# tsbertalan/openmg

Measured on AMD Instinct MI355X. Metric: V-cycles/sec, 3-D 7-point Poisson 256^3, higher is better.
Workload: dtype f64

## Files before the change

### include/openmg_hip.h

```cpp
#ifndef OPENMG_HIP_H
#define OPENMG_HIP_H

#include <stdint.h>

#ifdef __cplusplus
extern "C" {
#endif

#define OMG_OK                0
#define OMG_ERR_INVALID       1
#define OMG_ERR_NO_DEVICE     2
#define OMG_ERR_HIP           3
#define OMG_ERR_SINGULAR      4
#define OMG_ERR_NO_DIAGONAL   5
#define OMG_ERR_ALLOC         6
#define OMG_ERR_UNSUPPORTED   7

#define OMG_SMOOTH_GS_LEX     0
#define OMG_SMOOTH_GS_COLOUR  1
#define OMG_SMOOTH_JACOBI     2

typedef struct {
    int64_t n_rows, n_cols, nnz;
    const int32_t *indptr;
    const int32_t *indices;
    const double  *data;
} omg_csr;

typedef struct omg_hierarchy omg_hierarchy;
typedef struct omg_csr_result omg_csr_result;

const char *omg_last_error(void);
int omg_device_count(int *count);
int omg_set_device(int device);
int omg_device_mem_info(int64_t *free_bytes, int64_t *total_bytes);
int omg_device_synchronize(void);
const char *omg_version(void);

int omg_hierarchy_create(int n_levels, const omg_csr *A, const omg_csr *R,
                         int smoother, double omega, omg_hierarchy **out);
#define OMG_DTYPE_F64 0
#define OMG_DTYPE_F32 1
#define OMG_DTYPE_MIXED 2
int omg_hierarchy_create_ex(int n_levels, const omg_csr *A, const omg_csr *R, int smoother,
                            double omega, int dtype, omg_hierarchy **out);
int omg_hierarchy_create_from_fine(const omg_csr *A_in, int dim, const int64_t *shape, int n_restrictions, int smoother, double omega,
                                   int dtype, omg_hierarchy **out);

int omg_hierarchy_update_fine(omg_hierarchy *h, const double *data, int64_t nnz, int on_device);
int omg_hierarchy_dtype(const omg_hierarchy *h, int *dtype);
int omg_hierarchy_destroy(omg_hierarchy *h);
int omg_hierarchy_set_stream(omg_hierarchy *h, void *hip_stream);
int omg_hierarchy_sync(omg_hierarchy *h);
int omg_hierarchy_level_rows(const omg_hierarchy *h, int level, int64_t *n_rows);
int omg_hierarchy_level_sets(const omg_hierarchy *h, int level, int64_t *n_sets);
int omg_hierarchy_level_fused(const omg_hierarchy *h, int level, int *fused);
#define OMG_LEVEL_FUSED_LAST_SET   1
#define OMG_LEVEL_SCATTER_PROLONG  2
#define OMG_LEVEL_UNION_WALK       16
#define OMG_LEVEL_MARCH            32
#define OMG_LEVEL_MARCH_SCAN       512
#define OMG_LEVEL_PLANE            64
#define OMG_LEVEL_VAR7             256
#define OMG_LEVEL_STENCIL27        128
int omg_hierarchy_level_flags(const omg_hierarchy *h, int level, int *flags);
int omg_hierarchy_use_plane(omg_hierarchy *h, int enable);
#define OMG_CYCLE_V 0
#define OMG_CYCLE_F 1
#define OMG_CYCLE_W 2
int omg_hierarchy_set_cycle(omg_hierarchy *h, int shape, double over_correction);
int omg_hierarchy_get_cycle(const omg_hierarchy *h, int *shape, double *over_correction);
int omg_hierarchy_plane_info(const omg_hierarchy *h, int level, int64_t *out8);
int omg_hierarchy_set_info(const omg_hierarchy *h, int level, int set, int64_t *rows, int64_t *nnz);
#define OMG_FORMAT_FIELDS 12
int omg_hierarchy_format_info(const omg_hierarchy *h, int level, int op, int set, int64_t *out);
int omg_format_selftest(const omg_csr *A, int dtype, int64_t *out);

int omg_vcycle(omg_hierarchy *h, int level, const double *b, double *x,
               int pre, int post, double *norm);
int omg_vcycle_ex(omg_hierarchy *h, int level, const double *b, const double *x_in, double *x_out, double *x_pre,
                  int pre, int post, double *norm);

int omg_solve(omg_hierarchy *h, const double *b, double *x, int pre, int post,
              int max_cycles, double threshold, int *cycles_done, double *norm);

int omg_vcycle_dev(omg_hierarchy *h, int level, const double *b_dev, const double *x_in_dev, double *x_out_dev,
                   double *x_pre_dev, int pre, int post, double *norm);
int omg_resident_load_dev(omg_hierarchy *h, const double *b_dev, const double *x0_dev );
int omg_resident_fetch_dev(omg_hierarchy *h, double *x_dev);

int omg_hierarchy_cycle_dev(omg_hierarchy *h, const double *b_dev, double *x_dev, int pre, int post,
                            void *hip_stream);

int omg_resident_load(omg_hierarchy *h, const double *b, const double *x0 );
int omg_resident_cycle(omg_hierarchy *h, int pre, int post, double *norm );
int omg_resident_cycles(omg_hierarchy *h, int pre, int post, int n_cycles, double *norms );
int omg_resident_fetch(omg_hierarchy *h, double *x);
int omg_resident_spmv_time(omg_hierarchy *h, int reps, double *avg_ms);
int omg_resident_pcg(omg_hierarchy *h, int pre, int post, int max_iter, double threshold, int *iterations,
                     double *norms , double *true_norm, int *breakdown);
int omg_resident_use_graph(omg_hierarchy *h, int enable);

#define OMG_PROFILE_CLASSES 7
int omg_profile_enable(omg_hierarchy *h, int mask);
int omg_profile_read(omg_hierarchy *h, int64_t *launches, double *total_ms);

int omg_level_smooth(omg_hierarchy *h, int level, const double *b, double *x, int iterations);
int omg_level_residual(omg_hierarchy *h, int level, const double *b, const double *x,
                       double *r, double *norm );
int omg_level_spmv(omg_hierarchy *h, int level, const double *x, double *y);

int omg_level_restrict(omg_hierarchy *h, int level, const double *fine, double *coarse);
int omg_level_prolong_add(omg_hierarchy *h, int level, const double *coarse, double *fine_inout);
int omg_coarse_solve(omg_hierarchy *h, const double *b, double *x);
int omg_hierarchy_coarse_info(const omg_hierarchy *h, int64_t *out4);

int omg_spmv(const omg_csr *A, const double *x, double *y);
int omg_residual(const omg_csr *A, const double *b, const double *x, double *r, double *norm);
int omg_gauss_seidel(const omg_csr *A, const double *b, double *x, int smoother, double omega,
                     int iterations, double threshold, int *sweeps_done);
int omg_direct_solve(const omg_csr *A, const double *b, double *x);

int omg_rap(const omg_csr *R, const omg_csr *A, omg_csr_result **out,
            int64_t *n_rows, int64_t *n_cols, int64_t *nnz);
int omg_spgemm(const omg_csr *X, const omg_csr *Y, omg_csr_result **out,
               int64_t *n_rows, int64_t *n_cols, int64_t *nnz);
int omg_csr_result_fetch(omg_csr_result *res, int32_t *indptr, int32_t *indices, double *data);
int omg_csr_result_free(omg_csr_result *res);

int omg_restriction(int dim, const int64_t *shape, int32_t *indptr, int32_t *indices,
                    double *data, int64_t *n_rows, int64_t *nnz);

int omg_host_checksum(const void *buf, int64_t bytes, uint64_t *out);

typedef struct {
    omg_csr A;
    omg_csr R;
    int64_t n_halo;
    const int32_t *keys;
    int32_t n_sets;
    int32_t n_peers;
    const int32_t *peers;
    const int64_t *send_off;
    const int32_t *send_idx;
    const int64_t *recv_off;
    int32_t set_group;
    const int32_t *entry_group;
} omg_dist_level;
// ... 93 lines not shown
```

### openmg_amd/_hip.py

```python
import ctypes
import os

import numpy as np
import scipy.sparse as sp

_HERE = os.path.dirname(os.path.abspath(__file__))
LIB_PATH = os.environ.get("OMG_LIB_PATH") or os.path.join(_HERE, "lib", "libopenmg_hip.so")

OMG_OK = 0
ERR_INVALID, ERR_NO_DEVICE, ERR_HIP, ERR_SINGULAR, ERR_NO_DIAGONAL, ERR_ALLOC, ERR_UNSUPPORTED = range(1, 8)
SMOOTH_GS_LEX, SMOOTH_GS_COLOUR, SMOOTH_JACOBI = 0, 1, 2
PROFILE_CLASSES = 7
PROFILE_NAMES = ("smoother_set_sweep", "residual", "restrict", "prolong_add", "residual_norm", "plane_down", "plane_up")

SMOOTHERS = {
    "gs": SMOOTH_GS_LEX, "lex": SMOOTH_GS_LEX, "gauss-seidel": SMOOTH_GS_LEX, "gaussSeidel": SMOOTH_GS_LEX,
    "colour": SMOOTH_GS_COLOUR, "color": SMOOTH_GS_COLOUR, "rbgs": SMOOTH_GS_COLOUR,
    "red-black": SMOOTH_GS_COLOUR, "multicolour": SMOOTH_GS_COLOUR,
    "jacobi": SMOOTH_JACOBI, "weighted-jacobi": SMOOTH_JACOBI,
}


class HipError(RuntimeError):

    def __init__(self, code, message):
        super().__init__("libopenmg_hip: %s (code %d)" % (message, code))
        self.code = code


class CsrView(ctypes.Structure):
    _fields_ = [("n_rows", ctypes.c_int64), ("n_cols", ctypes.c_int64), ("nnz", ctypes.c_int64),
                ("indptr", ctypes.c_void_p), ("indices", ctypes.c_void_p), ("data", ctypes.c_void_p)]


_P = ctypes.c_void_p
_I = ctypes.c_int
_D = ctypes.c_double
_PP = ctypes.POINTER(ctypes.c_void_p)
_CSR = ctypes.POINTER(CsrView)
_I64P = ctypes.POINTER(ctypes.c_int64)
_IP = ctypes.POINTER(ctypes.c_int)
_DP = ctypes.POINTER(ctypes.c_double)

SIGNATURES = {
    "omg_last_error": (ctypes.c_char_p, []),
    "omg_version": (ctypes.c_char_p, []),
    "omg_device_count": (_I, [_IP]),
    "omg_set_device": (_I, [_I]),
    "omg_hierarchy_create": (_I, [_I, _CSR, _CSR, _I, _D, _PP]),
    "omg_hierarchy_create_ex": (_I, [_I, _CSR, _CSR, _I, _D, _I, _PP]),
    "omg_hierarchy_create_from_fine": (_I, [_CSR, _I, _I64P, _I, _I, _D, _I, _PP]),
    "omg_hierarchy_dtype": (_I, [_P, _IP]),
    "omg_hierarchy_update_fine": (_I, [_P, _P, ctypes.c_int64, _I]),
    "omg_hierarchy_destroy": (_I, [_P]),
    "omg_hierarchy_set_stream": (_I, [_P, _P]),
    "omg_hierarchy_sync": (_I, [_P]),
    "omg_hierarchy_level_rows": (_I, [_P, _I, _I64P]),
    "omg_hierarchy_level_sets": (_I, [_P, _I, _I64P]),
    "omg_hierarchy_set_info": (_I, [_P, _I, _I, _I64P, _I64P]),
    "omg_hierarchy_level_fused": (_I, [_P, _I, _IP]),
    "omg_hierarchy_level_flags": (_I, [_P, _I, _IP]),
    "omg_hierarchy_use_plane": (_I, [_P, _I]),
    "omg_hierarchy_set_cycle": (_I, [_P, _I, _D]),
    "omg_hierarchy_get_cycle": (_I, [_P, _IP, _DP]),
    "omg_hierarchy_plane_info": (_I, [_P, _I, _I64P]),
    "omg_hierarchy_format_info": (_I, [_P, _I, _I, _I, _I64P]),
    "omg_format_selftest": (_I, [_CSR, _I, _I64P]),
    "omg_vcycle": (_I, [_P, _I, _P, _P, _I, _I, _DP]),
    "omg_vcycle_ex": (_I, [_P, _I, _P, _P, _P, _P, _I, _I, _DP]),
    "omg_vcycle_dev": (_I, [_P, _I, _P, _P, _P, _P, _I, _I, _DP]),
    "omg_resident_load_dev": (_I, [_P, _P, _P]),
    "omg_resident_fetch_dev": (_I, [_P, _P]),
    "omg_device_synchronize": (_I, []),
    "omg_device_mem_info": (_I, [_I64P, _I64P]),
    "omg_solve": (_I, [_P, _P, _P, _I, _I, _I, _D, _IP, _DP]),
    "omg_resident_load": (_I, [_P, _P, _P]),
    "omg_resident_cycle": (_I, [_P, _I, _I, _DP]),
    "omg_resident_cycles": (_I, [_P, _I, _I, _I, _DP]),
    "omg_resident_fetch": (_I, [_P, _P]),
    "omg_resident_spmv_time": (_I, [_P, _I, _DP]),
    "omg_resident_use_graph": (_I, [_P, _I]),
    "omg_resident_pcg": (_I, [_P, _I, _I, _I, _D, _IP, _DP, _DP, _IP]),
    "omg_profile_enable": (_I, [_P, _I]),
    "omg_profile_read": (_I, [_P, _I64P, _DP]),
    "omg_level_smooth": (_I, [_P, _I, _P, _P, _I]),
    "omg_level_residual": (_I, [_P, _I, _P, _P, _P, _DP]),
    "omg_level_spmv": (_I, [_P, _I, _P, _P]),
    "omg_level_restrict": (_I, [_P, _I, _P, _P]),
    "omg_level_prolong_add": (_I, [_P, _I, _P, _P]),
    "omg_coarse_solve": (_I, [_P, _P, _P]),
    "omg_hierarchy_coarse_info": (_I, [_P, _I64P]),
    "omg_spmv": (_I, [_CSR, _P, _P]),
    "omg_residual": (_I, [_CSR, _P, _P, _P, _DP]),
    "omg_gauss_seidel": (_I, [_CSR, _P, _P, _I, _D, _I, _D, _IP]),
    "omg_direct_solve": (_I, [_CSR, _P, _P]),
    "omg_rap": (_I, [_CSR, _CSR, _PP, _I64P, _I64P, _I64P]),
    "omg_spgemm": (_I, [_CSR, _CSR, _PP, _I64P, _I64P, _I64P]),
    "omg_csr_result_fetch": (_I, [_P, _P, _P, _P]),
    "omg_csr_result_free": (_I, [_P]),
    "omg_restriction": (_I, [_I, _I64P, _P, _P, _P, _I64P, _I64P]),
    "omg_host_checksum": (_I, [_P, ctypes.c_int64, ctypes.POINTER(ctypes.c_uint64)]),
    "omg_dist_create": (_I, [_I, _I, _I, _P, _CSR, _I64P, _I, _D, _PP]),
    "omg_dist_create_ex": (_I, [_I, _I, _I, _P, _CSR, _I64P, _I, _D, _I, _PP]),
    "omg_dist_destroy": (_I, [_P]),
    "omg_dist_set_tail": (_I, [_P, _P]),
    "omg_hierarchy_cycle_dev": (_I, [_P, _P, _P, _I, _I, _P]),
    "omg_dist_set_stream": (_I, [_P, _P]),
    "omg_dist_sync": (_I, [_P]),
    "omg_rccl_unique_id": (_I, [_P]),
    "omg_rccl_self_exchange_time": (_I, [ctypes.c_int64, _I, _DP]),
    "omg_pdist_create": (_I, [_I, _I, _I, _I, _I, _I, _P, _D, _PP]),
    "omg_pdist_destroy": (_I, [_P]),
    "omg_pdist_set_tail": (_I, [_P, _P]),
    "omg_pdist_connect": (_I, [_P, _P, _P]),
    "omg_peer_access": (_I, [_I, _I, _P]),
    "omg_pdist_p2p_handle_count": (_I, [_P, _P]),
    "omg_pdist_p2p_handles": (_I, [_P, _P, _I]),
    "omg_pdist_p2p_open": (_I, [_P, _I, _P, _I]),
    "omg_pdist_p2p_local": (_I, [_P, _P]),
    "omg_pdist_p2p_enable": (_I, [_P, _I]),
    "omg_pdist_p2p_status": (_I, [_P, _P]),
    "omg_pdist_p2p_layout": (_I, [_P, _I64P, _I, _IP, _I]),
    "omg_pdist_cycles_squares": (_I, [_P, _I, _P]),
    "omg_pdist_rccl_ranks": (_I, [_P, _IP]),
    "omg_pdist_load": (_I, [_P, _P, _P]),
    "omg_pdist_fetch": (_I, [_P, _P]),
    "omg_pdist_sync": (_I, [_P]),
    "omg_pdist_info": (_I, [_P, _I64P]),
    "omg_pdist_set_gate": (_I, [_P, _I]),
    "omg_pdist_trace": (_I, [_P, _I]),
    "omg_pdist_progress": (_I, [_P, ctypes.POINTER(ctypes.c_uint)]),
    "omg_pdist_cycles": (_I, [_P, _I, _P]),
    "omg_pdist_cycles_ex": (_I, [_P, _I, _I, _I, _P]),
    "omg_pdist_group_cycles_ex": (_I, [_P, _I, _I, _I, _P]),
    "omg_sdist_p2p_handle_count": (_I, [_P, _P]),
    "omg_sdist_p2p_handles": (_I, [_P, _P, _I]),
    "omg_sdist_p2p_open": (_I, [_P, _I, _P, _I]),
    "omg_sdist_p2p_local": (_I, [_P, _P]),
    "omg_sdist_p2p_enable": (_I, [_P, _I]),
    "omg_sdist_p2p_status": (_I, [_P, _P]),
    "omg_sdist_p2p_layout": (_I, [_P, _I64P, _I, _IP]),
    "omg_pdist_group_create": (_I, [_I, _P, _PP]),
    "omg_pdist_group_destroy": (_I, [_P]),
    "omg_pdist_group_cycles": (_I, [_P, _I, _P]),
# ... 255 lines not shown
        check(lib().omg_resident_fetch_dev(self._h, ctypes.c_void_p(int(x_ptr))))

    def solve(self, b, x, pre, post, max_cycles, threshold):
        n = self.sizes[0]
        b = vec(b, n)
        assert x.dtype == np.float64 and x.flags.c_contiguous and x.size == n
        cycles = ctypes.c_int(0)
        norm = ctypes.c_double(0.0)
        check(lib().omg_solve(self._h, b.ctypes.data, x.ctypes.data, int(pre), int(post), int(max_cycles),
                              float(threshold), ctypes.byref(cycles), ctypes.byref(norm)))
        return cycles.value, norm.value

    def cycle_dev(self, b_dev, x_dev, pre, post, hip_stream=None):
        check(lib().omg_hierarchy_cycle_dev(self._h, ctypes.c_void_p(int(b_dev)), ctypes.c_void_p(int(x_dev)), int(pre), int(post),
                                            ctypes.c_void_p(hip_stream or 0)))

    def resident_load(self, b, x0=None):
        b = vec(b, self.sizes[0])
        x0 = None if x0 is None else vec(x0, self.sizes[0])
        check(lib().omg_resident_load(self._h, b.ctypes.data, None if x0 is None else x0.ctypes.data))

    def resident_cycle(self, pre, post, want_norm=True):
        if want_norm:
            norm = ctypes.c_double(0.0)
            check(lib().omg_resident_cycle(self._h, int(pre), int(post), ctypes.byref(norm)))
            return norm.value
        check(lib().omg_resident_cycle(self._h, int(pre), int(post), None))
        return None

    def resident_cycles(self, pre, post, n_cycles):
        norms = (ctypes.c_double * max(int(n_cycles), 1))()
        check(lib().omg_resident_cycles(self._h, int(pre), int(post), int(n_cycles), norms))
        return [float(norms[k]) for k in range(int(n_cycles))]

    def resident_fetch(self):
        x = np.empty(self.sizes[0], dtype=np.float64)
        check(lib().omg_resident_fetch(self._h, x.ctypes.data))
        return x

    def resident_pcg(self, pre, post, max_iter, threshold=0.0):
        max_iter = int(max_iter)
        if max_iter < 1:
            raise ValueError("max_iter must be >= 1")
        norms = np.zeros(max_iter, dtype=np.float64)
        it, tn, bd = ctypes.c_int(0), ctypes.c_double(0.0), ctypes.c_int(0)
        check(lib().omg_resident_pcg(self._h, int(pre), int(post), max_iter, float(threshold), ctypes.byref(it),
                                     norms.ctypes.data_as(_DP), ctypes.byref(tn), ctypes.byref(bd)))
        return int(it.value), norms[:it.value].copy(), float(tn.value), bool(bd.value)

    def spmv_time(self, reps=20):
        ms = ctypes.c_double(0.0)
        check(lib().omg_resident_spmv_time(self._h, int(reps), ctypes.byref(ms)))
        return ms.value

    def use_graph(self, enable=True):
        check(lib().omg_resident_use_graph(self._h, 1 if enable else 0))

    def set_stream(self, hip_stream):
        check(lib().omg_hierarchy_set_stream(self._h, ctypes.c_void_p(hip_stream or 0)))

    def sync(self):
        check(lib().omg_hierarchy_sync(self._h))

    def device_dtype(self):
        code = ctypes.c_int(-1)
        check(lib().omg_hierarchy_dtype(self._h, ctypes.byref(code)))
        return np.dtype(np.float32 if code.value in (DTYPE_F32, DTYPE_MIXED) else np.float64)

    def level_sets(self, level):
        v = ctypes.c_int64(0)
        check(lib().omg_hierarchy_level_sets(self._h, level, ctypes.byref(v)))
        return v.value

    def level_fused(self, level):
        v = ctypes.c_int(0)
        check(lib().omg_hierarchy_level_fused(self._h, level, ctypes.byref(v)))
        return bool(v.value)

    def level_flags(self, level):
        f = ctypes.c_int(0)
        check(lib().omg_hierarchy_level_flags(self._h, int(level), ctypes.byref(f)))
        return {"fused_last_set": bool(f.value & 1), "scatter_prolong": bool(f.value & 2), "union_walk": bool(f.value & 16),
                "march": bool(f.value & 32), "plane": bool(f.value & 64), "stencil27": bool(f.value & 128), "var7": bool(f.value & 256),
                "march_scan": bool(f.value & 512)}

    def use_plane(self, enable=True):
        check(lib().omg_hierarchy_use_plane(self._h, 1 if enable else 0))

    def set_cycle(self, shape="V", over_correction=1.0):
        check(lib().omg_hierarchy_set_cycle(self._h, cycle_code(shape), over_correction_of(over_correction)))

    def get_cycle(self):
        code, alpha = ctypes.c_int(-1), ctypes.c_double(0.0)
        check(lib().omg_hierarchy_get_cycle(self._h, ctypes.byref(code), ctypes.byref(alpha)))
        return {v: k for k, v in CYCLES.items()}[code.value], alpha.value

    PLANE_FIELDS = ("nx", "ny", "nz", "tile_x", "tile_y", "tile_z", "workgroups", "threads")

    def plane_info(self, level):
        out = (ctypes.c_int64 * len(self.PLANE_FIELDS))()
        check(lib().omg_hierarchy_plane_info(self._h, int(level), out))
        return dict(zip(self.PLANE_FIELDS, [int(v) for v in out]))

    def set_info(self, level, s):
        rows, nnz = ctypes.c_int64(0), ctypes.c_int64(0)
        check(lib().omg_hierarchy_set_info(self._h, level, s, ctypes.byref(rows), ctypes.byref(nnz)))
        return rows.value, nnz.value

    FORMAT_FIELDS = ("rows", "nnz", "blocks", "pattern_blocks", "pattern_rows", "pattern_nnz",
                     "coldict_nnz", "valdict_nnz", "format_bytes", "csr_bytes", "ell_blocks", "ell_nnz")

    def format_info(self, level, op="A", set=-1):
        out = (ctypes.c_int64 * len(self.FORMAT_FIELDS))()
        check(lib().omg_hierarchy_format_info(self._h, int(level), {"A": 0, "R": 1, "P": 2}[op], int(set), out))
        return dict(zip(self.FORMAT_FIELDS, [int(v) for v in out]))

    def profile_enable(self, classes=True):
        if classes is True:
            mask = -1
        elif not classes:
            mask = 0
        else:
            mask = 0
            for name in classes:
                mask |= 1 << PROFILE_NAMES.index(name)
        check(lib().omg_profile_enable(self._h, mask))

    def profile_read(self):
        n = (ctypes.c_int64 * PROFILE_CLASSES)()
        ms = (ctypes.c_double * PROFILE_CLASSES)()
        check(lib().omg_profile_read(self._h, n, ms))
        return {PROFILE_NAMES[i]: (int(n[i]), float(ms[i])) for i in range(PROFILE_CLASSES)}

    def smooth(self, level, b, x, iterations):
        n = self.sizes[level]
        b = vec(b, n)
        assert x.dtype == np.float64 and x.flags.c_contiguous and x.size == n
        check(lib().omg_level_smooth(self._h, level, b.ctypes.data, x.ctypes.data, int(iterations)))
        return x

    def residual(self, level, b, x, want_norm=False):
        n = self.sizes[level]
        b, x = vec(b, n), vec(x, n)
        r = np.empty(n)
        if want_norm:
            norm = ctypes.c_double(0.0)
            check(lib().omg_level_residual(self._h, level, b.ctypes.data, x.ctypes.data, r.ctypes.data, ctypes.byref(norm)))
            return r, norm.value
        check(lib().omg_level_residual(self._h, level, b.ctypes.data, x.ctypes.data, r.ctypes.data, None))
        return r

    def spmv(self, level, x):
        n = self.sizes[level]
        x = vec(x, n)
        y = np.empty(n)
        check(lib().omg_level_spmv(self._h, level, x.ctypes.data, y.ctypes.data))
        return y

    def restrict(self, level, fine):
        fine = vec(fine, self.sizes[level])
        out = np.empty(self.sizes[level + 1])
        check(lib().omg_level_restrict(self._h, level, fine.ctypes.data, out.ctypes.data))
        return out

    def prolong_add(self, level, coarse, fine):
        coarse = vec(coarse, self.sizes[level + 1])
        out = vec(fine, self.sizes[level], copy=True)
# ... 105 lines not shown
```

### openmg_amd/csrc/coarse.hip

```cpp
#include <algorithm>
#include <cmath>
#include <cstdlib>
#include <type_traits>

#include "common.h"

namespace omg {
namespace {

constexpr int64_t LDS_DOUBLES = 6144;

int grid1d(int64_t n, int cap = 65536) {
    int64_t g = (n + 255) / 256;
    if (g > cap) g = cap;
    if (g < 1) g = 1;
    return (int)g;
}

__device__ __forceinline__ double wsum(double v) {
#pragma unroll
    for (int off = 32; off > 0; off >>= 1) v += __shfl_down(v, off, 64);
    return v;
}
__device__ __forceinline__ float wsum(float v) {
#pragma unroll
    for (int off = 32; off > 0; off >>= 1) v += __shfl_down(v, off, 64);
    return v;
}

__global__ void couple_kernel(const double *B, int64_t m, const int32_t *cptr, const int32_t *cidx,
                              const double *cval, int64_t g, double *T) {
    const int64_t tot = m * g;
    for (int64_t t = blockIdx.x * (int64_t)blockDim.x + threadIdx.x; t < tot; t += (int64_t)gridDim.x * blockDim.x) {
        const int64_t i = t / g, c = t % g;
        double acc = 0.0;
        for (int32_t p = cptr[c]; p < cptr[c + 1]; ++p) acc += B[i * m + cidx[p]] * cval[p];
        T[t] = acc;
    }
}

__global__ void schur_kernel(const int32_t *rptr, const int32_t *ridx, const double *rval, int64_t g,
                             const double *T, double *S, int64_t ld) {
    const int64_t tot = g * g;
    for (int64_t t = blockIdx.x * (int64_t)blockDim.x + threadIdx.x; t < tot; t += (int64_t)gridDim.x * blockDim.x) {
        const int64_t q = t / g, c = t % g;
        double acc = 0.0;
        for (int32_t p = rptr[q]; p < rptr[q + 1]; ++p) acc += rval[p] * T[int64_t(ridx[p]) * g + c];
        if (acc != 0.0) S[q * ld + c] -= acc;
    }
}

template <typename V>
__global__ void narrow_kernel(const double *src, V *dst, int64_t n) {
    for (int64_t i = blockIdx.x * (int64_t)blockDim.x + threadIdx.x; i < n; i += (int64_t)gridDim.x * blockDim.x)
        dst[i] = V(src[i]);
}

template <typename V>
__global__ __launch_bounds__(256) void interior_solve_kernel(const V *__restrict__ binv, const int64_t *__restrict__ binv_off,
                                                             const int64_t *__restrict__ blk_off,
                                                             const int32_t *__restrict__ wg_blk, const int32_t *__restrict__ wg_row,
                                                             const int32_t *__restrict__ perm, const V *__restrict__ b,
                                                             V *__restrict__ y) {
    const int k = wg_blk[blockIdx.x];
    const int64_t o = blk_off[k], m = blk_off[k + 1] - o;
    const int64_t i = wg_row[blockIdx.x] + (threadIdx.x >> 6);
    if (i >= m) return;
    const int lane = threadIdx.x & 63;
    const V *row = binv + binv_off[k] + i * m;
    V acc = V(0);
    for (int64_t j = lane; j < m; j += 64) acc += row[j] * b[perm[o + j]];
    acc = wsum(acc);
    if (lane == 0) y[o + i] = acc;
}

template <typename V>
__global__ __launch_bounds__(256) void separator_solve_kernel(const V *__restrict__ sinv, int64_t g, int64_t n_int,
                                                              const int32_t *__restrict__ gptr, const int32_t *__restrict__ gidx,
                                                              const V *__restrict__ gval, const int32_t *__restrict__ perm,
                                                              const V *__restrict__ b, const V *__restrict__ y,
                                                              V *__restrict__ xg, V *__restrict__ x) {
    extern __shared__ unsigned char s_raw[];
    V *s_rhs = reinterpret_cast<V *>(s_raw);
    for (int64_t q = threadIdx.x; q < g; q += 256) {
        V acc = V(0);
        for (int32_t p = gptr[q]; p < gptr[q + 1]; ++p) acc += gval[p] * y[gidx[p]];
        s_rhs[q] = b[perm[n_int + q]] - acc;
    }
// ... 15 lines not shown
                                                               const int32_t *__restrict__ iptr, const int32_t *__restrict__ iidx,
                                                               const V *__restrict__ ival, const V *__restrict__ xg,
                                                               const int32_t *__restrict__ perm, const V *__restrict__ y,
                                                               int64_t w, V *__restrict__ x) {
    extern __shared__ unsigned char s_raw[];
    V *s_t = reinterpret_cast<V *>(s_raw);
    const int k = wg_blk[blockIdx.x];
    const int64_t o = blk_off[k], m = blk_off[k + 1] - o;
    const int64_t head = min(w, m), tail0 = max(head, m - w);
    const int64_t nt = head + (m - tail0);
    for (int64_t c = threadIdx.x; c < nt; c += 256) {
        const int64_t j = c < head ? c : tail0 + (c - head);
        V acc = V(0);
        for (int32_t p = iptr[o + j]; p < iptr[o + j + 1]; ++p) acc += ival[p] * xg[iidx[p]];
        s_t[c] = acc;
    }
    __syncthreads();
    const int64_t i = wg_row[blockIdx.x] + (threadIdx.x >> 6);
    if (i >= m) return;
    const int lane = threadIdx.x & 63;
    const V *row = binv + binv_off[k] + i * m;
    V acc = V(0);
    for (int64_t c = lane; c < nt; c += 64) {
        const int64_t j = c < head ? c : tail0 + (c - head);
        acc += row[j] * s_t[c];
    }
    acc = wsum(acc);
    if (lane == 0) x[perm[o + i]] = y[o + i] - acc;
}

constexpr int CHAIN_ROWS = 16;
template <typename V, bool BACK>
__global__ __launch_bounds__(256) void chain_step_kernel(const V *__restrict__ dinv, int64_t m, int64_t r0, const int32_t *__restrict__ ptr,
                                                         const int32_t *__restrict__ idx, const V *__restrict__ val,
                                                         const V *__restrict__ b, const V *src, V *z, V *x, int last) {
    extern __shared__ unsigned char s_raw[];
    V *s_t = reinterpret_cast<V *>(s_raw);
    for (int64_t q = threadIdx.x; q < m; q += 256) {
        V acc = V(0);
        for (int32_t p = ptr[r0 + q]; p < ptr[r0 + q + 1]; ++p) acc += val[p] * src[idx[p]];
        s_t[q] = BACK ? acc : b[r0 + q] - acc;
    }
    __syncthreads();
    const int lane = threadIdx.x & 63;
    const int64_t q0 = int64_t(blockIdx.x) * CHAIN_ROWS + (threadIdx.x >> 6) * 4;
    V acc[4] = {V(0), V(0), V(0), V(0)};
    const V *row[4];
#pragma unroll
    for (int r = 0; r < 4; ++r) row[r] = dinv + min(q0 + r, m - 1) * m;
    for (int64_t j = lane; j < m; j += 64) {
        const V t = s_t[j];
#pragma unroll
        for (int r = 0; r < 4; ++r) acc[r] += row[r][j] * t;
    }
#pragma unroll
    for (int r = 0; r < 4; ++r) {
        const V v = wsum(acc[r]);
        if (lane == 0 && q0 + r < m) {
            if (BACK) x[r0 + q0 + r] = z[r0 + q0 + r] - v;
            else { z[r0 + q0 + r] = v; if (last) x[r0 + q0 + r] = v; }
        }
    }
}

struct HostSub {
    std::vector<int32_t> ptr, idx;
    std::vector<double> val;
};

template <typename T, typename Al>
void put(DevBuf<T> &d, const std::vector<T, Al> &h, hipStream_t s) {
    d.alloc(std::max<size_t>(h.size(), 1));
    d.upload(h.data(), h.size(), s);
}

template <typename V>
void put_values(DevBuf<V> &d, const std::vector<double> &h, hipStream_t s, std::vector<V> &keep) {
    keep.assign(h.begin(), h.end());
    d.alloc(std::max<size_t>(keep.size(), 1));
    d.upload(keep.data(), keep.size(), s);
}

constexpr int SINE_THREADS = 1024;
typedef double v4d __attribute__((ext_vector_type(4)));
template <typename V, int E>
__global__ __launch_bounds__(SINE_THREADS) void sine_solve_kernel(const V *__restrict__ b, V *__restrict__ x, int nx, int ny, int nz,
                                                                 const double *__restrict__ tables, const double *__restrict__ lambda) {
    extern __shared__ double sine_buf[];
    const int px = nx + 1, n = nx * ny * nz;
    double *const lt = sine_buf + ((px * ny * nz + 1) & ~1);
    const int nt = (nx + ny + nz) * E;
    for (int r = int(threadIdx.x); r < nt; r += SINE_THREADS) lt[r] = tables[r];
    constexpr int PER = 8192 / SINE_THREADS;
    int place[PER];
    double lam[PER];
#pragma unroll
    for (int q = 0; q < PER; ++q) {
        const int r = int(threadIdx.x) + q * SINE_THREADS;
        place[q] = r < n ? (r / nx) * px + r % nx : -1;
        lam[q] = r < n ? lambda[r] : 1.0;
        if (r < n) sine_buf[place[q]] = double(b[r]);
    }
    __syncthreads();
    const int lane = int(threadIdx.x) & 63, wave = int(threadIdx.x) >> 6;
    const int c16 = lane & 15, k4 = lane >> 4;
#pragma unroll 1
    for (int pass = 0; pass < 6; ++pass) {
        const int axis = pass % 3;
        const int ne = axis == 0 ? nx : axis == 1 ? ny : nz;
        const int n_lines = n / ne;
        const int da = axis == 0 ? 1 : nx, sb = axis == 0 ? 0 : 1;
        const int sa = axis == 0 ? px : axis == 1 ? ny * px : px;
        const int stride = axis == 0 ? 1 : axis == 1 ? px : ny * px;
        const double *S = lt + (axis == 0 ? 0 : axis == 1 ? nx : nx + ny) * E;
        if (pass == 3) {
#pragma unroll
            for (int q = 0; q < PER; ++q)
                if (place[q] >= 0) sine_buf[place[q]] = sine_buf[place[q]] / lam[q];
            __syncthreads();
        }
        if (ne <= 1) continue;
        const int n_blocks = (n_lines + 15) >> 4, k_steps = (ne + 3) >> 2;
#pragma unroll 1
        for (int bl = wave; bl < n_blocks; bl += SINE_THREADS / 64) {
            const int line = 16 * bl + c16;
            const bool live = line < n_lines;
            const int bs = live ? (line / da) * sa + (line % da) * sb : 0;
            v4d acc[E / 16];
#pragma unroll
            for (int ib = 0; ib < E / 16; ++ib) acc[ib] = v4d{0.0, 0.0, 0.0, 0.0};
            double bvs[E / 4], avs[E / 16][E / 4];
#pragma unroll
            for (int ks = 0; ks < E / 4; ++ks) {
                const int k = 4 * ks + k4;
                bvs[ks] = (live && k < ne) ? sine_buf[bs + k * stride] : 0.0;
#pragma unroll
                for (int ib = 0; ib < E / 16; ++ib) avs[ib][ks] = S[(16 * ib + c16) * E + k];
            }
#pragma unroll
            for (int ks = 0; ks < E / 4; ++ks)
#pragma unroll
                for (int ib = 0; ib < E / 16; ++ib)
                    if (ks < k_steps) acc[ib] = __builtin_amdgcn_mfma_f64_16x16x4f64(avs[ib][ks], bvs[ks], acc[ib], 0, 0, 0);
            if (live) {
#pragma unroll
                for (int ib = 0; ib < E / 16; ++ib)
#pragma unroll
                    for (int r = 0; r < 4; ++r) {
                        const int i = 16 * ib + 4 * r + k4;
                        if (i < ne) sine_buf[bs + i * stride] = acc[ib][r];
                    }
            }
        }
        __syncthreads();
    }
#pragma unroll
    for (int q = 0; q < PER; ++q)
        if (place[q] >= 0) x[int(threadIdx.x) + q * SINE_THREADS] = V(sine_buf[place[q]]);
}

__device__ __forceinline__ void wave_lds_exchange() {
    __builtin_amdgcn_fence(__ATOMIC_RELEASE, "wavefront");
    __builtin_amdgcn_wave_barrier();
    __builtin_amdgcn_fence(__ATOMIC_ACQUIRE, "wavefront");
}

template <typename V>
__global__ __launch_bounds__(SINE_THREADS) void sine_cube16_kernel(const V *__restrict__ b, V *__restrict__ x, const double *__restrict__ tables,
                                                                   const double *__restrict__ lambda) {
    constexpr int N = 16, PX = N + 1;
    __shared__ double buf[N * N * PX];
    const int lane = int(threadIdx.x) & 63, w = int(threadIdx.x) >> 6;
    const int c = lane & 15, k4 = lane >> 4;
    double sx[4], sy[4], sz[4], lam[4], rhs[4];
#pragma unroll
    for (int ks = 0; ks < 4; ++ks) {
        sx[ks] = tables[(0 * N + c) * N + 4 * ks + k4];
        sy[ks] = tables[(1 * N + c) * N + 4 * ks + k4];
        sz[ks] = tables[(2 * N + c) * N + 4 * ks + k4];
        rhs[ks] = double(b[(w * N + c) * N + 4 * ks + k4]);
        lam[ks] = lambda[((4 * ks + k4) * N + w) * N + c];
    }
    auto transform = [&](const double (&S)[4], const double (&in)[4]) -> v4d {
        v4d acc = {0.0, 0.0, 0.0, 0.0};
#pragma unroll
        for (int ks = 0; ks < 4; ++ks) acc = __builtin_amdgcn_mfma_f64_16x16x4f64(S[ks], in[ks], acc, 0, 0, 0);
        return acc;
    };
    double in[4];
    v4d acc = transform(sx, rhs);
#pragma unroll
    for (int r = 0; r < 4; ++r) buf[(w * N + c) * PX + 4 * r + k4] = acc[r];
    wave_lds_exchange();
#pragma unroll
    for (int ks = 0; ks < 4; ++ks) in[ks] = buf[(w * N + 4 * ks + k4) * PX + c];
    acc = transform(sy, in);
#pragma unroll
    for (int r = 0; r < 4; ++r) buf[(w * N + 4 * r + k4) * PX + c] = acc[r];
    __syncthreads();
#pragma unroll
    for (int ks = 0; ks < 4; ++ks) in[ks] = buf[((4 * ks + k4) * N + w) * PX + c];
    acc = transform(sz, in);
#pragma unroll
    for (int r = 0; r < 4; ++r) in[r] = acc[r] / lam[r];
    acc = transform(sz, in);
#pragma unroll
    for (int r = 0; r < 4; ++r) buf[((4 * r + k4) * N + w) * PX + c] = acc[r];
    __syncthreads();
#pragma unroll
    for (int ks = 0; ks < 4; ++ks) in[ks] = buf[(w * N + c) * PX + 4 * ks + k4];
    acc = transform(sx, in);
#pragma unroll
    for (int r = 0; r < 4; ++r) buf[(w * N + c) * PX + 4 * r + k4] = acc[r];
    wave_lds_exchange();
#pragma unroll
    for (int ks = 0; ks < 4; ++ks) in[ks] = buf[(w * N + 4 * ks + k4) * PX + c];
    acc = transform(sy, in);
#pragma unroll
    for (int r = 0; r < 4; ++r) x[(w * N + 4 * r + k4) * N + c] = V(acc[r]);
}

bool detect_symmetric_star(const HostCsr &A, int64_t &nx, int64_t &ny, int64_t &nz, double (&c)[4]) {
    const int64_t n = A.n_rows;
    if (n < 2) return false;
    auto has = [&](int64_t r, int64_t col) {
        for (int32_t p = A.indptr[r]; p < A.indptr[r + 1]; ++p)
            if (A.indices[p] == col) return true;
        return false;
    };
    nx = n;
    for (int64_t r = 1; r < n; ++r)
        if (!has(r, r - 1)) { nx = r; break; }
    if (nx < 2 || n % nx) return false;
    const int64_t lines = n / nx;
    ny = lines;
    for (int64_t q = 1; q < lines; ++q)
        if (!has(q * nx, (q - 1) * nx)) { ny = q; break; }
    if (lines % ny) return false;
    nz = lines / ny;
    const int64_t sj = nx, sk = nx * ny;
    bool have[4] = {false, false, false, false};
    c[0] = c[1] = c[2] = c[3] = 0.0;
    for (int64_t r = 0; r < n; ++r) {
        const int64_t i = r % nx, jl = (r / nx) % ny, kl = r / sk;
        const int want = 1 + (i > 0) + (i + 1 < nx) + (jl > 0) + (jl + 1 < ny) + (kl > 0) + (kl + 1 < nz);
        if (A.indptr[r + 1] - A.indptr[r] != want) return false;
        int seen = 0;
        for (int32_t p = A.indptr[r]; p < A.indptr[r + 1]; ++p) {
            const int64_t off = int64_t(A.indices[p]) - r;
            int slot, bit;
            if (off == 0) { slot = 0; bit = 1; }
            else if (off == -1 && i > 0) { slot = 1; bit = 2; }
            else if (off == 1 && i + 1 < nx) { slot = 1; bit = 4; }
            else if (off == -sj && jl > 0 && ny > 1) { slot = 2; bit = 8; }
            else if (off == sj && jl + 1 < ny) { slot = 2; bit = 16; }
            else if (off == -sk && kl > 0 && nz > 1) { slot = 3; bit = 32; }
            else if (off == sk && kl + 1 < nz) { slot = 3; bit = 64; }
            else return false;
            if (seen & bit) return false;
            seen |= bit;
            if (!have[slot]) { have[slot] = true; c[slot] = A.data[p]; }
            else if (A.data[p] != c[slot]) return false;
        }
    }
    return have[0];
}

}

template <typename V>
void CoarseSolver<V>::build(const HostCsr &A, hipStream_t s) {
    OMG_REQUIRE(A.n_rows == A.n_cols, "coarse operator must be square");
    n = A.n_rows;
    if (n == 0) return;
    {
        const char *e = getenv("OMG_COARSE_BLOCKS"), *q = getenv("OMG_COARSE_SINE");
        if (!(e && atoi(e) > 0) && !(q && q[0] == '0') && build_sine(A, s)) return;
    }
    int64_t band = 0;
    for (int64_t i = 0; i < n; ++i)
        for (int32_t p = A.indptr[i]; p < A.indptr[i + 1]; ++p) band = std::max<int64_t>(band, std::llabs(int64_t(A.indices[p]) - i));
    w = std::max<int64_t>(band, 1);
    const int64_t lds_cap = LDS_DOUBLES * int64_t(sizeof(double) / sizeof(V));
    P = 1;
    {
        const char *e = getenv("OMG_COARSE_BLOCKS");
        const int forced = e ? atoi(e) : 0;
        const bool big = double(n) * double(n) * sizeof(V) > double(size_t(256) << 20);
        double best = double(n) * double(n);
        if (forced > 1 || (forced == 0 && big))
            for (int q = 2; q <= 64; ++q) {
                const int64_t gq = int64_t(q - 1) * w;
                if (gq >= n || gq > lds_cap || 2 * w > lds_cap) break;
                const int64_t mq = (n - gq + q - 1) / q;
                if (mq < 2 * w) break;
                const double cost = double(q) * double(mq) * double(mq) + double(gq) * double(gq);
                if ((forced == q) || (forced == 0 && cost < best)) { best = cost; P = q; }
                if (forced == q) break;
            }
    }
    std::vector<int32_t> plain_ptr(A.indptr.begin(), A.indptr.end());
    DevBuf<int32_t> d_ptr, d_idx;
// ... 196 lines not shown
    DevBuf<double> c_val, r_val;
    for (int k = 0; k < K; ++k) {
        const int64_t r0 = int64_t(k) * bs, m = std::min(n, r0 + bs) - r0;
        if (k > 0) for (int64_t i = r0 - bs; i < r0; ++i) rmap[size_t(i)] = -1;
        for (int64_t i = 0; i < m; ++i) rmap[size_t(r0 + i)] = int32_t(i);
        d_rmap.upload(rmap.data(), size_t(n), s);
        OMG_HIP(hipStreamSynchronize(s));
        fill_augmented_from_csr(d_ptr, d_idx, d_val, n, d_rmap.p, d_rmap.p, m, W.p, s);
        if (k > 0) {
            const int64_t p0 = r0 - bs, mp = bs;
            HostSub col, row;
            std::vector<std::vector<std::pair<int32_t, double>>> cols{size_t(m)};
            for (int64_t r = p0; r < r0; ++r)
                for (int32_t p = up.ptr[size_t(r)]; p < up.ptr[size_t(r) + 1]; ++p) cols[size_t(up.idx[size_t(p)] - r0)].emplace_back(int32_t(r - p0), up.val[size_t(p)]);
            col.ptr.assign(size_t(m) + 1, 0);
            for (int64_t c = 0; c < m; ++c) {
                for (auto &e : cols[size_t(c)]) { col.idx.push_back(e.first); col.val.push_back(e.second); }
                col.ptr[size_t(c) + 1] = int32_t(col.idx.size());
            }
            row.ptr.assign(size_t(m) + 1, 0);
            for (int64_t q = 0; q < m; ++q) {
                for (int32_t p = lo.ptr[size_t(r0 + q)]; p < lo.ptr[size_t(r0 + q) + 1]; ++p) { row.idx.push_back(int32_t(lo.idx[size_t(p)] - p0)); row.val.push_back(lo.val[size_t(p)]); }
                row.ptr[size_t(q) + 1] = int32_t(row.idx.size());
            }
            put(c_ptr, col.ptr, s); put(c_idx, col.idx, s); put(c_val, col.val, s);
            put(r_ptr, row.ptr, s); put(r_idx, row.idx, s); put(r_val, row.val, s);
            hipLaunchKernelGGL(couple_kernel, dim3(grid1d(mp * m)), dim3(256), 0, s, inv64.p, mp, c_ptr.p, c_idx.p, c_val.p, m, T.p);
            hipLaunchKernelGGL(schur_kernel, dim3(grid1d(m * m)), dim3(256), 0, s, r_ptr.p, r_idx.p, r_val.p, m, T.p, W.p, 2 * m);
            OMG_HIP(hipGetLastError());
        }
        gauss_jordan_inverse(W.p, m, inv64.p, s, keep.p);
        hipLaunchKernelGGL((narrow_kernel<V>), dim3(grid1d(m * m)), dim3(256), 0, s, inv64.p, dinv.p + size_t(k) * size_t(bs) * size_t(bs), m * m);
        OMG_HIP(hipGetLastError());
        OMG_HIP(hipStreamSynchronize(s));
    }
    if (lds_need > size_t(48) << 10) {
        OMG_HIP(hipFuncSetAttribute(reinterpret_cast<const void *>(chain_step_kernel<V, false>), hipFuncAttributeMaxDynamicSharedMemorySize, int(lds_need)));
        OMG_HIP(hipFuncSetAttribute(reinterpret_cast<const void *>(chain_step_kernel<V, true>), hipFuncAttributeMaxDynamicSharedMemorySize, int(lds_need)));
    }
    bytes = (size_t(2 * K - 1) * size_t(bs) * size_t(bs)) * sizeof(V);
}

template <typename V>
bool CoarseSolver<V>::build_sine(const HostCsr &A, hipStream_t s) {
    int64_t gx = 0, gy = 0, gz = 0;
    double c[4];
    if (A.n_rows > 8192 || !detect_symmetric_star(A, gx, gy, gz, c) || gx > 32 || gy > 32 || gz > 32) return false;
    const double pi = 3.14159265358979323846264338327950288;
    const int64_t E = std::max(gx, std::max(gy, gz)) <= 16 ? 16 : 32;
    std::vector<double> tab(size_t((gx + gy + gz) * E), 0.0), lam(size_t(A.n_rows));
    auto table = [&](double *t, int64_t m) {
        const long double f = std::sqrt(2.0L / (long double)(m + 1));
        for (int64_t i = 0; i < m; ++i)
            for (int64_t p = 0; p < m; ++p)
                t[i * E + p] = m == 1 ? 1.0 : double(f * sinl((long double)pi * (long double)((i + 1) * (p + 1)) / (long double)(m + 1)));
    };
    table(tab.data(), gx);
    table(tab.data() + gx * E, gy);
    table(tab.data() + (gx + gy) * E, gz);
    double smallest = 1e300, largest = 0.0;
    for (int64_t r = 0; r < A.n_rows; ++r) {
        const int64_t p = r % gx, q = (r / gx) % gy, t = r / (gx * gy);
        double l = c[0] + 2.0 * c[1] * std::cos(pi * double(p + 1) / double(gx + 1));
        if (gy > 1) l += 2.0 * c[2] * std::cos(pi * double(q + 1) / double(gy + 1));
        if (gz > 1) l += 2.0 * c[3] * std::cos(pi * double(t + 1) / double(gz + 1));
        lam[size_t(r)] = l;
        smallest = std::min(smallest, std::fabs(l));
        largest = std::max(largest, std::fabs(l));
    }
    if (!(smallest > 1e-13 * largest)) return false;
    P = 0;
    sx = int(gx); sy = int(gy); sz = int(gz);
    sine.alloc(tab.size());
    lambda.alloc(lam.size());
    sine.upload(tab.data(), tab.size(), s);
    lambda.upload(lam.data(), lam.size(), s);
    OMG_HIP(hipStreamSynchronize(s));
    w = gx * gy;
    bytes = (tab.size() + lam.size()) * sizeof(double);
    return true;
}

template <typename V>
void CoarseSolver<V>::solve(const V *b, V *x, hipStream_t s) const {
    if (n == 0) return;
    if (P == 0) {
        const int E = std::max(sx, std::max(sy, sz)) <= 16 ? 16 : 32;
        const size_t lds = (size_t(sx + 1) * size_t(sy) * size_t(sz) + 2 + size_t(sx + sy + sz) * size_t(E)) * sizeof(double);
        static const bool cube16 = [] { const char *e = experiment_env("OMG_SINE_CUBE16"); return !(e && e[0] == '0'); }();
        if (E == 16 && sx == 16 && sy == 16 && sz == 16 && cube16) {
            hipLaunchKernelGGL((sine_cube16_kernel<V>), dim3(1), dim3(SINE_THREADS), 0, s, b, x, sine.p, lambda.p);
        } else if (E == 16) {
            hipLaunchKernelGGL((sine_solve_kernel<V, 16>), dim3(1), dim3(SINE_THREADS), lds, s, b, x, sx, sy, sz, sine.p, lambda.p);
        } else {
            if (lds > size_t(64) * 1024)
                OMG_HIP(hipFuncSetAttribute(reinterpret_cast<const void *>(sine_solve_kernel<V, 32>), hipFuncAttributeMaxDynamicSharedMemorySize, int(lds)));
            hipLaunchKernelGGL((sine_solve_kernel<V, 32>), dim3(1), dim3(SINE_THREADS), lds, s, b, x, sx, sy, sz, sine.p, lambda.p);
        }
        OMG_HIP(hipGetLastError());
        return;
    }
    if (P == 1) {
        launch_dense_gemv<V>(inv.p, b, x, n, s);
        return;
    }
    if (P == -1) {
        for (int k = 0; k < K; ++k) {
            const int64_t r0 = int64_t(k) * bs, m = std::min(n, r0 + bs) - r0;
            hipLaunchKernelGGL((chain_step_kernel<V, false>), dim3(unsigned((m + CHAIN_ROWS - 1) / CHAIN_ROWS)), dim3(256), size_t(m) * sizeof(V), s,
                               dinv.p + size_t(k) * size_t(bs) * size_t(bs), m, r0, lo_ptr.p, lo_idx.p, lo_val.p, b, z.p, z.p, x, k == K - 1 ? 1 : 0);
        }
        for (int k = K - 2; k >= 0; --k) {
            const int64_t r0 = int64_t(k) * bs;
            hipLaunchKernelGGL((chain_step_kernel<V, true>), dim3(unsigned((bs + CHAIN_ROWS - 1) / CHAIN_ROWS)), dim3(256), size_t(bs) * sizeof(V), s,
                               dinv.p + size_t(k) * size_t(bs) * size_t(bs), bs, r0, up_ptr.p, up_idx.p, up_val.p, b, x, z.p, x, 0);
        }
        OMG_HIP(hipGetLastError());
        return;
    }
    hipLaunchKernelGGL((interior_solve_kernel<V>), dim3((unsigned)n_wg), dim3(256), 0, s, binv.p, binv_off.p, blk_off.p,
                       wg_blk.p, wg_row.p, perm.p, b, y.p);
    hipLaunchKernelGGL((separator_solve_kernel<V>), dim3((unsigned)((g + 3) / 4)), dim3(256), (size_t)(g) * sizeof(V), s,
                       sinv.p, g, n_int, gi_ptr.p, gi_idx.p, gi_val.p, perm.p, b, y.p, xg.p, x);
    hipLaunchKernelGGL((interior_correct_kernel<V>), dim3((unsigned)n_wg), dim3(256), (size_t)(2 * w) * sizeof(V), s, binv.p,
                       binv_off.p, blk_off.p, wg_blk.p, wg_row.p, ig_ptr.p, ig_idx.p, ig_val.p, xg.p, perm.p, y.p, w, x);
    OMG_HIP(hipGetLastError());
}

template struct CoarseSolver<double>;
template struct CoarseSolver<float>;

}
```

### openmg_amd/csrc/common.h

```cpp
#pragma once
#include <hip/hip_runtime.h>

#include <algorithm>
#include <array>
#include <cstdint>
#include <cstdio>
#include <cstdlib>
#include <cstring>
#include <new>
#include <stdexcept>
#include <memory>
#include <string>
#include <type_traits>
#include <utility>
#include <vector>

#include "../../include/openmg_hip.h"

#if !defined(OMG_EXPERIMENTS) && (defined(PLANE_STORE_AUX) || defined(PLANE_LA_BIG) || defined(PLANE_LA) || defined(PLANE_WAVE_SYNC) || \
                                  defined(PLANE_WSYNC_F32) || defined(S27_COEF_AUX) || defined(S27_SG) || defined(S27_WAVES) ||        \
                                  defined(MARCH_NAP_MAX) || defined(OMG_ROWBLK_NNZ) || defined(PLANE_SETPRIO))
#error "tuning switches are experiments: add -DOMG_EXPERIMENTS"
#endif

// ... 395 lines not shown
};

template <typename V>
struct RowArgsT {
    const V *x = nullptr;
    const V *b = nullptr;
    V *y = nullptr;
    double omega = 1.0;
    double *partials = nullptr;
    V *zero = nullptr;
    const int32_t *ymap = nullptr;
    const V *first_diag = nullptr;
    int first_end = 0;
    bool first_jacobi = false;
    const RowValues<V> *values = nullptr;
};
using RowArgs = RowArgsT<double>;

template <typename V>
void launch_rows(const DevCsrT<V> &A, int mode, int set, const RowArgsT<V> &args, hipStream_t s);
template <typename V>
void launch_rows_range(const DevCsrT<V> &A, int mode, int set_begin, int set_end, const RowArgsT<V> &args,
                       hipStream_t s);
template <typename V>
void launch_gs_serial(const DevCsrT<V> &A, int set_begin, int set_end, const RowArgsT<V> &args,
                      hipStream_t s);
constexpr int SUM_FOLD = 64;
void launch_sum(double *partials, int64_t n, double *out, hipStream_t s);
void launch_sum_sqrt(double *partials, int64_t n, double *out, hipStream_t s);
void launch_sum_batch(const double *partials, int64_t stride, int64_t n, int count, double *out, bool take_sqrt,
                      hipStream_t s);
template <typename S, typename D>
void launch_gather(const S *src, const int32_t *idx, D *dst, int64_t n, hipStream_t s);
template <typename S, typename D>
void launch_scatter(const S *src, const int32_t *idx, D *dst, int64_t n, hipStream_t s);
template <typename V>
void launch_diagonal(const DevCsrT<V> &A, V *diag, hipStream_t s);
template <typename V>
void launch_scale_values(const V *in, V *out, int64_t n, double factor, hipStream_t s);
template <typename V>
void launch_first_relaxation(const V *b, const V *diag, V *x, int64_t n, int64_t first_end, bool jacobi, double omega,
                             hipStream_t s);
template <typename V>
void launch_dense_gemv(const V *M, const V *v, V *out, int64_t n, hipStream_t s);
template <typename V>
void launch_dense_gemv_rows(const V *M, const V *v, V *out, int64_t rows, int64_t n,
                            hipStream_t s);
void dense_inverse_from_csr(const DevCsr &A, double *Minv, hipStream_t s);
void gauss_jordan_inverse(double *W, int64_t n, double *Minv, hipStream_t s, double *keep_ws = nullptr);
void fill_augmented_from_csr(const int32_t *indptr, const int32_t *indices, const double *data, int64_t n_rows,
                             const int32_t *rmap, const int32_t *cmap, int64_t m, double *W, hipStream_t s);

template <typename V>
struct CoarseSolver {
    int64_t n = 0;
    int P = 1;
    DevBuf<V> inv;
    int64_t n_int = 0, g = 0, w = 0;
    DevBuf<V> binv, sinv;
    DevBuf<int64_t> blk_off, binv_off;
    DevBuf<int32_t> perm;
    DevBuf<int32_t> wg_blk, wg_row;
    int64_t n_wg = 0;
    DevBuf<int32_t> gi_ptr, gi_idx;
    DevBuf<V> gi_val;
    DevBuf<int32_t> ig_ptr, ig_idx;
    DevBuf<V> ig_val;
    DevBuf<V> y, xg;
    int sx = 0, sy = 0, sz = 0;
    DevBuf<double> sine, lambda;
    size_t bytes = 0;
    bool retain_workspace = false;
    DevBuf<double> ws_aug, ws_inv64, ws_keep;
    int64_t bs = 0;
    int K = 0;
    DevBuf<V> dinv;
    DevBuf<int32_t> lo_ptr, lo_idx, up_ptr, up_idx;
    DevBuf<V> lo_val, up_val;
    DevBuf<V> z;
    void build_chain(const HostCsr &A, const int32_t *d_ptr, const int32_t *d_idx, const double *d_val, hipStream_t s);
    void build(const HostCsr &A, hipStream_t s);
    bool build_sine(const HostCsr &A, hipStream_t s);
    void solve(const V *b, V *x, hipStream_t s) const;
};

constexpr int MARCH_FACE_PAD = 72;
struct MarchGeom {
    int nx = 0, ny = 0, nz = 0;
    int TJ = 0, TK = 0;
    int ntj = 0, ntk = 0, n_tiles = 0;
    int T = 0, n_grp = 0;
    int n_pat = 0;
};
template <typename V>
struct MarchPlan {
    MarchGeom g;
    DevBuf<uint32_t> codes;
    DevBuf<V> coef;
    DevBuf<uint32_t> sync;
    DevBuf<int32_t> order;
    DevBuf<V> faceJ, faceK;
    bool line1 = false;
    DevBuf<V> tri;
    bool per_row = false;
    DevBuf<V> rowc;
    bool line_scan = false;
    int scan_c = 0, scan_g = 0;
    DevBuf<uint8_t> rowcode;
    DevBuf<V> face_scan;
    bool build(const omg_csr &A, hipStream_t s);
    void sweep(V *x, const V *b, hipStream_t s) const;
    bool timed_out(hipStream_t s) const;
};

struct DevCsrPlain {
    int64_t n_rows = 0, n_cols = 0, nnz = 0;
    DevBuf<int32_t> indptr, indices;
    DevBuf<double> data;
};
void galerkin_chain_device(const omg_csr &A0, int dim, const int64_t *shape, int n_restrictions, std::vector<DevCsrPlain> &A,
                           std::vector<DevCsrPlain> &R, hipStream_t s);
HostCsr download_csr(const DevCsrPlain &M, hipStream_t s);
bool rap_aggregation_device(const DevCsrPlain &R, const DevCsrPlain &A, DevCsrPlain &C, hipStream_t s);

bool is_plain_aggregation(const omg_csr &R, int64_t nx, int64_t ny, int64_t nz, double &w);

constexpr int PLANE_EDGE = 4;
struct PlaneGeom {
    int nx = 0, ny = 0, nz = 0;
    int hx = 0;
    int z_base = 0, z_end = 0, kv0 = 0, kv1 = 0, kc_off = 0, nzc = 0;
    int TX = 0, TY = 0, LZ = 0;
    int PX = 0, PY = 0;
    int ntx = 0, nty = 0, ntz = 0, n_wg = 0;
    int threads = 0;
    size_t lds_bytes = 0;
    double c[7] = {0, 0, 0, 0, 0, 0, 0};
    double w = 0.0;
    double over = 1.0;
    bool dim2 = false;
    bool jacobi = false;
    double omega = 1.0;
    bool block = false;
    bool la2 = true;
};
template <typename V>
struct PlanePlan {
    PlaneGeom g;
    DevBuf<double> partials;
    uint32_t *status = nullptr;
    bool build(const omg_csr &A, const omg_csr &R, Ordering &ord, bool jacobi = false, double omega = 1.0);
    bool build_device(const DevCsrPlain &A, int nx, int ny, int nz, double w, Ordering &ord, bool jacobi, double omega, hipStream_t s);
    bool finish_geometry(int64_t nx, int64_t ny, int64_t nz, const double (&c)[7], double w, bool jacobi, double omega);
    void spmv(const V *x, V *y, hipStream_t s) const;
    HostCsr operator_csr() const;
    HostCsr restriction_csr() const;
    void build_slab(int nx, int ny, int nz_own, int ghost, int ghost_c, bool first, bool last, const double (&c)[7], double w);
    struct Peer {
        V *x[2] = {nullptr, nullptr};
        V *bc[2] = {nullptr, nullptr};
        int64_t shift = 0, cshift = 0;
        int planes = 0, cplanes = 0;
        int zc_lo = 0, zc_hi = 0;
        const uint32_t *wait_flag[4] = {nullptr, nullptr, nullptr, nullptr};
        uint32_t wait_seq[4] = {0, 0, 0, 0};
        bool fused_wait = true;
        uint32_t *done = nullptr;
        uint32_t *flag[2] = {nullptr, nullptr};
        uint32_t seq = 0;
        uint32_t *status = nullptr;
        uint32_t spin = 1u << 21;
    };
    struct Coarse {
        const int32_t *map = nullptr;
        V *b = nullptr;
        V *x = nullptr;
        const V *diag = nullptr;
        int first_end = 0;
        const V *e = nullptr;
    };
    void tune(V *x, V *tmp, const V *b, const Coarse &c, hipStream_t s, bool finest = true);
    float time_pair(V *x, V *tmp, const V *b, const Coarse &c, hipStream_t s, bool finest, int pairs);
    enum { PART_ALL = 0, PART_EDGE = 1, PART_INNER = 2 };
    bool can_split() const {
        return !g.dim2 && !g.block && !(g.la2 && g.threads <= 128) && (g.z_end - g.z_base) >= 3 * PLANE_EDGE;
    }
    int split_partials() const {
        const int nzo = g.z_end - g.z_base;
        return nzo >= 3 * PLANE_EDGE ? g.ntx * g.nty * (2 + (nzo - 2 * PLANE_EDGE + g.LZ - 1) / g.LZ) : g.n_wg;
    }
    struct Gate {
        const uint32_t *flag[4] = {nullptr, nullptr, nullptr, nullptr};
        uint32_t seq[4] = {0, 0, 0, 0};
        uint32_t *status = nullptr;
        uint32_t spin = 1u << 21;
    };
    bool can_gate() const { return can_split() && 2 * g.ntx * g.nty <= 192 && (g.z_end - g.z_base) >= 96; }
    int gate_lz() const;
    int gate_partials() const;
    void down(const V *x_old, V *x_new, const V *b, bool x_zero, const Coarse &c, hipStream_t s, const Peer *peer = nullptr,
              bool sweep = true, int part = PART_ALL, const Gate *gate = nullptr) const;
    void up(const V *x_old, V *x_new, const V *b, const Coarse &c, double *out, hipStream_t s, const Peer *peer = nullptr,
            bool sweep = true, int part = PART_ALL, const Gate *gate = nullptr) const;
};

template <typename V>
struct Var7Plan {
    int nx = 0, ny = 0, nz = 0;
    double w = 0.0;
    double over = 1.0;
    bool sym = false;
    int tx = 0, ty = 0, lz = 0, ntx = 0, nty = 0, ntz = 0, threads = 0;
    int64_t n_wg = 0;
    DevBuf<V> cD, cM[3], cP[3];
    DevBuf<double> partials;
    bool build(const omg_csr &A, const omg_csr &R, Ordering &ord, hipStream_t s);
    bool build_device(const DevCsrPlain &A, int nx, int ny, int nz, double w, Ordering &ord, hipStream_t s);
    HostCsr operator_csr(hipStream_t s) const;
    HostCsr restriction_csr() const;
    struct Coarse {
        const int32_t *map = nullptr;
        V *b = nullptr;
        const V *e = nullptr;
    };
    void down(const V *x_old, V *x_new, const V *b, bool x_zero, const Coarse &c, hipStream_t s, bool sweep = true) const;
    void up(const V *x_old, V *x_new, const V *b, const Coarse &c, double *out, hipStream_t s, bool sweep = true) const;
    void rap_from(const int32_t *indptr, const double *vals, bool write_fine, double *coarse_dense, Var7Plan<V> *coarse,
                  unsigned long long *err, hipStream_t s);
};

template <typename V>
void var7_rap(const int32_t *indptr, const double *vals, int nx, int ny, int nz, double w, Var7Plan<V> *fine, Var7Plan<V> *coarse,
              double *coarse_dense, unsigned long long *err, hipStream_t s);

struct S27Geom {
    int nx = 0, ny = 0, nz = 0;
    int hx = 0, hy = 0, hz = 0;
    int64_t na = 0;
    int rg = 0;
    int L = 0, G = 0;
    int64_t nl = 0, ng = 0;
    int wpb = 4;
    int n_wg = 0;
    double w = 0.0;
    double over = 1.0;
};
template <typename V>
struct Stencil27Plan {
    S27Geom g;
    DevBuf<V> coef;
    DevBuf<V> res67;
    DevBuf<double> partials;
    bool have67 = false;
    int64_t live_lo = 0, live_hi = 0, live_lo01 = 0, live_hi01 = 0;
    bool build(const omg_csr &A, const omg_csr &R, Ordering &ord, hipStream_t s);
    bool build_device(const DevCsrPlain &A, int nx, int ny, int nz, double w, Ordering &ord, hipStream_t s);
    void build_slab(const DevCsrPlain &A, int nx, int ny, int nz_ext, bool first, bool last, double w, hipStream_t s);
    bool tile(const DevCsrPlain &A, const S27Geom &q, int kz_lo, int kz_hi, int kb_lo, int kb_hi, hipStream_t s);
    size_t plane_rows_count() const;
    void pack_plane_rows(int K, V *buf, hipStream_t s) const;
    void unpack_plane_rows(int K, const V *buf, hipStream_t s);
    void sweep(const V *x_old, V *x_new, const V *b, bool x_zero, double *norm_old, bool last, double *norm_new, hipStream_t s);
    void place_tiles(V *x, V *tmp, V *b, hipStream_t s);
    void residual_restrict(const V *x, const V *b, bool use67, const int32_t *cmap, V *bc, hipStream_t s);
    void norm(const V *x, const V *b, bool use67, double *out, hipStream_t s);
    void prolong(V *x, const V *e, const int32_t *cmap, hipStream_t s);
    HostCsr operator_csr(hipStream_t s) const;
    HostCsr restriction_csr() const;
    void rap_from(const int32_t *indptr, const double *vals, bool write_fine, double *coarse_dense, Stencil27Plan<V> *coarse, hipStream_t s);
};

enum { PCG_RHO = 0, PCG_ALPHA = 1, PCG_BETA = 2, PCG_DONE = 3, PCG_BREAK = 4, PCG_ITERS = 5, PCG_NSC = 8 };
constexpr int PCG_MAX_WG = 2048;
struct PcgPlane {
    int nx, ny, nz, hx;
    int64_t nr;
    double c[7];
};
template <typename V>
int pcg_wgs(int64_t n);
template <typename V, typename Z>
void pcg_dots(const V *r, const Z *z, const V *q, int64_t n, double *part, const double *sc, hipStream_t s);
template <typename V>
void pcg_dot(const V *a, const V *b, int64_t n, double *part, const double *sc, hipStream_t s);
template <typename V, typename Z>
void pcg_pupdate(const Z *z, const V *p, V *p2, int64_t n, const double *sc, hipStream_t s);
template <typename V, typename Z>
void pcg_update(V *x, const V *p, V *r, const V *q, Z *rlo, int64_t n, double *part, const double *sc, hipStream_t s);
template <typename V, typename Z>
// ... 14 lines not shown
```

### openmg_amd/csrc/hierarchy.hip

```cpp
#include <algorithm>
#include <chrono>
#include <cmath>
#include <cstring>
#include <memory>
#include <array>
#include <map>
#include <mutex>
#include <thread>
#include <type_traits>

#include "common.h"

namespace omg {

std::vector<ScatteredBlock> &scattered_registry() {
    static std::vector<ScatteredBlock> r;
    return r;
}
static std::mutex &scattered_mutex() {
    static std::mutex m;
    return m;
}
static void scattered_release(ScatteredBlock &blk, size_t mapped) {
    auto report = [](const char *what, hipError_t e) {
// ... 81 lines not shown
                    "no HIP device visible: libopenmg_hip.so has no CPU fallback "
                    "(hipGetDeviceCount: " + std::string(hipGetErrorString(e)) + ")");
}

namespace {

inline bool getenv_flag(const char *name) { const char *e = getenv(name); return e && e[0] == '1'; }
inline bool getenv_flag0(const char *name) { const char *e = getenv(name); return e && e[0] == '0'; }

struct SweepStep {
    int set_begin, set_end;
    bool serial;
};

template <typename V>
struct Level {
    int64_t n = 0;
    DevCsrT<V> A;
    DevCsrT<V> R;
    DevCsrT<V> P;
    Ordering ord;
    DevBuf<int32_t> perm;
    DevBuf<int32_t> r_out;
    DevBuf<V> x, b, r, tmp;
    DevBuf<V> diag;
    DevBuf<double> partials;
    DevBuf<double> nat;
    V *xp = nullptr, *tp = nullptr;
    std::vector<SweepStep> plan;
    bool scatter_prolong = false;
    DevBuf<V> pw_data, pw_vdict, pw_pval, pw_vell;
    RowValues<V> pw;
    double pw_factor = 0.0;
    std::unique_ptr<MarchPlan<V>> march;
    std::unique_ptr<PlanePlan<V>> plane;
    std::unique_ptr<Stencil27Plan<V>> s27;
    std::unique_ptr<Var7Plan<V>> var7;
    DevBuf<char> pool;
    size_t pool_span = 0, pool_off1 = 0, pool_off2 = 0;
    DevBuf<V> spmv_y;
    bool format_pending = false;
};

struct ProfEvent {
    int cls;
    hipEvent_t a, b;
};

template <typename V>
struct Hier {
    using value_type = V;
    std::vector<Level<V>> lv;
    CoarseSolver<V> coarse;
    DevBuf<double> norm_dev;
    DevBuf<uint32_t> plane_status;
    DevBuf<V> pre_buf;
    int pre_level = -1;
    DevBuf<double> norms_dev;
    DevBuf<double> batch_partials;
    DevBuf<V> pcg_b, pcg_x, pcg_p, pcg_p2, pcg_q;
    DevBuf<double> pcg_sc, pcg_part, pcg_norms;
    bool mixed = false;
    struct Mixed {
        bool plane = false;
        PcgPlane pg{};
        DevCsrT<double> A;
        DevBuf<int32_t> src;
        DevBuf<double> b, x, x2, r, p, p2, q;
    } mx;
    int smoother = OMG_SMOOTH_GS_LEX;
    double omega = 1.0;
    int cycle_shape = OMG_CYCLE_V;
    double over = 1.0;
    hipStream_t own = nullptr, stream = nullptr;
    DevBuf<int32_t> indptr0;
    int64_t nnz0 = 0;
    std::vector<DevBuf<double>> dense27;
    bool upd7 = false;
    int g7[3] = {0, 0, 0};
    std::vector<DevBuf<double>> dense7;
    bool resident = false;
    bool no_fuse = [] { const char *e = getenv("OMG_NO_FUSE"); return e && e[0] == '1'; }();
    bool no_plane = false;
    struct GraphSlot {
        hipGraphExec_t exec = nullptr;
        int pre = -1, post = -1;
        std::vector<V *> before, after;
    };
    bool want_graph = false;
    std::vector<GraphSlot> graphs;
    unsigned profiling = 0;
    std::vector<ProfEvent> events;
    int64_t prof_n[OMG_PROFILE_CLASSES] = {0};
    double prof_ms[OMG_PROFILE_CLASSES] = {0};
    std::vector<hipEvent_t> event_pool;

    Hier() = default;
    Hier(const Hier &) = delete;
    Hier &operator=(const Hier &) = delete;
    ~Hier() {
        for (auto &g : graphs) if (g.exec) (void)hipGraphExecDestroy(g.exec);
        for (auto &e : events) { (void)hipEventDestroy(e.a); (void)hipEventDestroy(e.b); }
        for (auto &e : event_pool) (void)hipEventDestroy(e);
        if (own) (void)hipStreamDestroy(own);
    }
};

}
}

struct omg_hierarchy {
    std::unique_ptr<omg::Hier<double>> d;
    std::unique_ptr<omg::Hier<float>> f;
};

namespace omg {
namespace {

void check_diagonal(const omg_csr &A, int level) {
    const int64_t bad = first_row_without_diagonal(A);
    if (bad >= 0)
        throw Error(OMG_ERR_NO_DIAGONAL, "level " + std::to_string(level) + ": row " +
                                             std::to_string(bad) + " has no nonzero diagonal entry");
}

omg_csr view(const HostCsr &A) {
    return omg_csr{A.n_rows, A.n_cols, A.nnz, A.indptr.data(), A.indices.data(), A.data.data()};
}

template <typename V>
void order_level(Level<V> &L, const omg_csr &A, int smoother, hipStream_t s) {
    L.march.reset();
    if (smoother == OMG_SMOOTH_GS_LEX && !getenv_flag0("OMG_MARCH")) {
        std::unique_ptr<MarchPlan<V>> plan(new MarchPlan<V>);
        if (plan->build(A, s)) {
            L.march = std::move(plan);
            L.ord = Ordering();
            L.ord.identity = true;
            L.ord.sets = {0, A.n_rows};
            return;
        }
    }
    L.ord = make_ordering(A, smoother);
}

template <typename V>
void build_plan(Level<V> &L) {
    L.plan.clear();
    const int ns = (int)L.A.n_sets();
    int s = 0;
    while (s < ns) {
        auto one_block = [&](int k) { return L.A.set_blk[k + 1] - L.A.set_blk[k] == 1; };
        if (one_block(s)) {
            int e = s + 1;
            while (e < ns && one_block(e)) ++e;
            L.plan.push_back({s, e, e - s >= 2});
            s = e;
        } else {
            L.plan.push_back({s, s + 1, false});
            ++s;
        }
    }
}

template <typename V>
struct Prof {
    Hier<V> *h;
    int idx = -1;
    Prof(Hier<V> *hh, int level, int cls) : h(hh) {
        if (level != 0 || !((h->profiling >> cls) & 1u)) return;
// ... 320 lines not shown
    }
    L.x.zero(h->stream); L.tmp.zero(h->stream); L.b.zero(h->stream); C.x.zero(h->stream);
    L.xp = L.x.p;
    L.tp = L.tmp.p;
    OMG_HIP(hipStreamSynchronize(h->stream));
}

template <typename V>
void place_s27_tiles(Hier<V> *h) {
    if (h->lv.size() < 2) return;
    Level<V> &L = h->lv[0];
    if (!L.s27 || !L.tmp.p || L.n < POOL_TRIAL_MIN) return;
    L.s27->place_tiles(L.x.p, L.tmp.p, L.b.p, h->stream);
    L.x.zero(h->stream); L.tmp.zero(h->stream); L.b.zero(h->stream);
    OMG_HIP(hipStreamSynchronize(h->stream));
}

template <typename V>
void ensure_spmv_y(Hier<V> *h, Level<V> &L) {
    if (L.spmv_y.p) return;
    L.spmv_y.alloc(size_t(L.n));
    static const int trials = [] { const char *e = getenv("OMG_SPMV_TRIALS"); return e && e[0] ? atoi(e) : 16; }();
    if (trials < 2 || !L.plane || L.n < POOL_TRIAL_MIN) return;
    hipEvent_t e0, e1;
    OMG_HIP(hipEventCreate(&e0));
    OMG_HIP(hipEventCreate(&e1));
    auto timed = [&]() -> float {
        L.plane->spmv(L.xp, L.spmv_y.p, h->stream);
        OMG_HIP(hipEventRecord(e0, h->stream));
        for (int r = 0; r < 8; ++r) L.plane->spmv(L.xp, L.spmv_y.p, h->stream);
        OMG_HIP(hipEventRecord(e1, h->stream));
        OMG_HIP(hipEventSynchronize(e1));
        float ms = 0.0f;
        OMG_HIP(hipEventElapsedTime(&ms, e0, e1));
        return 1e3f * ms / 8.0f;
    };
    float best = timed(), worst = best;
    const bool debug = SetupTimer::on();
    if (debug) fprintf(stderr, "[omg setup] SpMV destination, candidate 0: %.1f us per launch\n", best);
    std::vector<DevBuf<V>> held;
    for (int k = 1; k < trials; ++k) {
        if (2.0 * double(sizeof(V)) * double(L.n) / (double(best) * 1e-6) >= 5.15e12) break;
        DevBuf<V> alt;
        try { alt.alloc(size_t(L.n), 0, pool_placement(k)); } catch (const Error &) { (void)hipGetLastError(); break; }
        std::swap(L.spmv_y, alt);
        const float t = timed();
        if (debug) fprintf(stderr, "[omg setup] SpMV destination, candidate %d (placement %d): %.1f us per launch\n", k, pool_placement(k), t);
        worst = std::max(worst, t);
        if (t < best) best = t;
        else std::swap(L.spmv_y, alt);
        held.push_back(std::move(alt));
    }
    (void)hipEventDestroy(e0);
    (void)hipEventDestroy(e1);
}

template <typename V>
bool use_s27(const Hier<V> *h, const Level<V> &L) {
    return L.s27 && !h->no_plane;
}

template <typename V>
bool use_var7(const Hier<V> *h, const Level<V> &L) {
    return L.var7 && !h->no_plane;
}

template <typename V>
bool use_plane(const Hier<V> *h, const Level<V> &L, int pre, int post) {
    (void)pre; (void)post;
    return L.plane && !h->no_plane;
}

template <typename V>
int cycle_body(Hier<V> *h, int l, int pre, int post, bool want_norm = false, double *pre_slot = nullptr,
               bool first_done = false, double *post_slot = nullptr, bool x_zero = false, int shape = -1);

template <typename V>
void cycle_children(Hier<V> *h, int l, int pre, int post, int shape, bool first_done, bool x_zero) {
    cycle_body(h, l + 1, pre, post, false, nullptr, first_done, nullptr, x_zero, shape);
    if (shape != OMG_CYCLE_V && l + 1 < (int)h->lv.size() - 1)
        cycle_body(h, l + 1, pre, post, false, nullptr, false, nullptr, false, shape == OMG_CYCLE_F ? OMG_CYCLE_V : OMG_CYCLE_W);
}

template <typename V>
int cycle_body(Hier<V> *h, int l, int pre, int post, bool want_norm, double *pre_slot, bool first_done, double *post_slot, bool x_zero,
               int shape) {
    if (shape < 0) shape = h->cycle_shape;
    const int last = (int)h->lv.size() - 1;
    if (l >= last) {
        coarse_solve_level(h);
        return NORM_NONE;
    }
    Level<V> &L = h->lv[l];
    Level<V> &C = h->lv[l + 1];
    if (use_s27(h, L)) {
        Stencil27Plan<V> &P = *L.s27;
        const bool child_zero = l + 1 < last && ((use_s27(h, C) && pre >= 1) || (use_plane(h, C, pre, post) && pre == 1));
        bool zero_now = x_zero;
        if (x_zero && pre == 0) {
            OMG_HIP(hipMemsetAsync(L.xp, 0, size_t(L.n) * sizeof(V), h->stream));
            zero_now = false;
        }
        for (int it = 0; it < pre; ++it) {
            Prof<V> p(h, l, 0);
            P.sweep(L.xp, L.tp, L.b.p, zero_now, (it == 0 && !zero_now) ? pre_slot : nullptr, it + 1 == pre, nullptr, h->stream);
            std::swap(L.xp, L.tp);
            zero_now = false;
        }
        if (l == h->pre_level) OMG_HIP(hipMemcpyAsync(h->pre_buf.p, L.xp, size_t(L.n) * sizeof(V), hipMemcpyDeviceToDevice, h->stream));
        if (l + 1 < last && !child_zero) OMG_HIP(hipMemsetAsync(C.xp, 0, size_t(C.n) * sizeof(V), h->stream));
        {
            Prof<V> p(h, l, 1);
            P.residual_restrict(L.xp, L.b.p, pre >= 1, L.r_out.p, C.b.p, h->stream);
        }
        cycle_children(h, l, pre, post, shape, false, child_zero);
        {
            Prof<V> p(h, l, 3);
            P.prolong(L.xp, C.xp, L.r_out.p, h->stream);
        }
        double *nslot = want_norm ? (post_slot ? post_slot : P.partials.p) : nullptr;
        for (int it = 0; it < post; ++it) {
            Prof<V> p(h, l, 0);
            const bool fin = it + 1 == post && want_norm;
            P.sweep(L.xp, L.tp, L.b.p, false, nullptr, fin, fin ? nslot : nullptr, h->stream);
            std::swap(L.xp, L.tp);
        }
        return want_norm ? NORM_S27 : NORM_NONE;
    }
    static const int halves = [] { const char *e = experiment_env("OMG_PLANE_HALVES"); return (e && (e[0] == '1' || e[0] == '2')) ? e[0] - '0' : 3; }();
    if (use_plane(h, L, pre, post) && halves == 2 && !x_zero && pre >= 1 && post >= 1) {
        const bool res_done = smooth_level(h, l, pre, FUSE_RESIDUAL, nullptr, first_done);
        residual_level(h, l, L.r.p, res_done);
        if (l + 1 < last) ensure_format(h, l + 1);
        const bool child_first = l + 1 < last && first_sweep_in_restrict(h, C, pre);
        restrict_level<V>(h, l, L.r.p, C.b.p, l + 1 < last ? C.xp : nullptr, child_first);
        cycle_children(h, l, pre, post, shape, child_first, false);
        typename PlanePlan<V>::Coarse c;
        c.map = L.r_out.p;
        c.e = C.xp;
        double *out = (want_norm && post == 1) ? (post_slot ? post_slot : L.plane->partials.p) : nullptr;
        L.plane->up(L.xp, L.tp, L.b.p, c, out, h->stream);
        std::swap(L.xp, L.tp);
        if (post > 1)
            return smooth_level(h, l, post - 1, want_norm ? FUSE_NORM : FUSE_NONE, nullptr, false, post_slot) ? NORM_LAST_SET : NORM_NONE;
        return out ? NORM_PLANE : NORM_NONE;
    }
    if (use_plane(h, L, pre, post) && halves == 1 && pre >= 1 && post >= 1) {
        if (pre > 1) smooth_level(h, l, pre - 1, FUSE_NONE, nullptr, first_done);
        if (l + 1 < last) ensure_format(h, l + 1);
        const bool child_first = l + 1 < last && first_sweep_in_restrict(h, C, pre);
        typename PlanePlan<V>::Coarse c;
        c.map = L.r_out.p;
        c.b = C.b.p;
        c.x = l + 1 < last ? C.xp : nullptr;
        c.diag = child_first ? C.diag.p : nullptr;
        c.first_end = child_first ? int(C.A.sets[1]) : 0;
        L.plane->down(L.xp, L.tp, L.b.p, x_zero, c, h->stream);
        std::swap(L.xp, L.tp);
        cycle_children(h, l, pre, post, shape, child_first, false);
        prolong_add_level<V>(h, l, C.xp, L.xp, h->over);
        return smooth_level(h, l, post, want_norm ? FUSE_NORM : FUSE_NONE, nullptr, false, post_slot) ? NORM_LAST_SET : NORM_NONE;
    }
    if (use_plane(h, L, pre, post)) {
        if (pre > 1) smooth_level(h, l, pre - 1, FUSE_NONE, nullptr, first_done);
        const bool child_plane = l + 1 < last && use_plane(h, C, pre, post);
        const bool child_zero = child_plane && pre <= 1 && halves == 3;
        if (l + 1 < last && !child_zero) ensure_format(h, l + 1);
        const bool child_first = l + 1 < last && !child_zero && !use_s27(h, C) && !L.plane->g.dim2 && first_sweep_in_restrict(h, C, pre);
        typename PlanePlan<V>::Coarse c;
        c.map = L.r_out.p;
        c.b = C.b.p;
        c.x = (l + 1 < last && !child_zero) ? C.xp : nullptr;
        c.diag = child_first ? C.diag.p : nullptr;
        c.first_end = child_first ? int(C.A.sets[1]) : 0;
        if (child_zero && pre == 0) OMG_HIP(hipMemsetAsync(C.xp, 0, size_t(C.n) * sizeof(V), h->stream));
        {
            Prof<V> p(h, l, 5);
            L.plane->down(L.xp, L.tp, L.b.p, x_zero, c, h->stream, nullptr, pre >= 1);
        }
        if (pre >= 1) std::swap(L.xp, L.tp);
        if (l == h->pre_level) OMG_HIP(hipMemcpyAsync(h->pre_buf.p, L.xp, size_t(L.n) * sizeof(V), hipMemcpyDeviceToDevice, h->stream));
        cycle_children(h, l, pre, post, shape, child_first, child_zero);
        c.e = C.xp;
        double *out = (want_norm && post <= 1) ? (post_slot ? post_slot : L.plane->partials.p) : nullptr;
        {
            Prof<V> p(h, l, 6);
            L.plane->up(L.xp, L.tp, L.b.p, c, out, h->stream, nullptr, post >= 1);
        }
        std::swap(L.xp, L.tp);
        if (post > 1)
            return smooth_level(h, l, post - 1, want_norm ? FUSE_NORM : FUSE_NONE, nullptr, false, post_slot) ? NORM_LAST_SET : NORM_NONE;
        return out ? NORM_PLANE : NORM_NONE;
    }
    if (use_var7(h, L)) {
        Var7Plan<V> &P = *L.var7;
        if (pre > 1) smooth_level(h, l, pre - 1, FUSE_NONE, nullptr, first_done);
        const bool child_zero = l + 1 < last && ((use_var7(h, C) && pre == 1) || (use_plane(h, C, pre, post) && pre == 1) || (use_s27(h, C) && pre >= 1));
        if (l + 1 < last && !child_zero) {
            if (!use_s27(h, C)) ensure_format(h, l + 1);
            OMG_HIP(hipMemsetAsync(C.xp, 0, size_t(C.n) * sizeof(V), h->stream));
        }
        typename Var7Plan<V>::Coarse c;
        c.map = L.r_out.p;
        c.b = C.b.p;
        {
            Prof<V> p(h, l, 5);
            P.down(L.xp, L.tp, L.b.p, x_zero && pre == 1, c, h->stream, pre >= 1);
        }
        if (pre >= 1) std::swap(L.xp, L.tp);
        else if (x_zero) OMG_HIP(hipMemsetAsync(L.xp, 0, size_t(L.n) * sizeof(V), h->stream));
        if (l == h->pre_level) OMG_HIP(hipMemcpyAsync(h->pre_buf.p, L.xp, size_t(L.n) * sizeof(V), hipMemcpyDeviceToDevice, h->stream));
        cycle_children(h, l, pre, post, shape, false, child_zero);
        c.e = C.xp;
        double *out = (want_norm && post <= 1) ? (post_slot ? post_slot : P.partials.p) : nullptr;
        {
            Prof<V> p(h, l, 6);
            P.up(L.xp, L.tp, L.b.p, c, out, h->stream, post >= 1);
        }
        std::swap(L.xp, L.tp);
        if (post > 1)
            return smooth_level(h, l, post - 1, want_norm ? FUSE_NORM : FUSE_NONE, nullptr, false, post_slot) ? NORM_LAST_SET : NORM_NONE;
        return out ? NORM_VAR7 : NORM_NONE;
    }
    const bool res_done = smooth_level(h, l, pre, FUSE_RESIDUAL, pre_slot, first_done);
    if (l == h->pre_level) OMG_HIP(hipMemcpyAsync(h->pre_buf.p, L.xp, size_t(L.n) * sizeof(V), hipMemcpyDeviceToDevice, h->stream));
    residual_level(h, l, L.r.p, res_done);
    const bool child_zero = l + 1 < last && ((use_plane(h, C, pre, post) && pre == 1 && halves == 3) || (use_s27(h, C) && pre >= 1));
    if (l + 1 < last && !child_zero && !use_s27(h, C)) ensure_format(h, l + 1);
    const bool child_first = l + 1 < last && !child_zero && !use_s27(h, C) && !use_var7(h, C) && first_sweep_in_restrict(h, C, pre);
    restrict_level<V>(h, l, L.r.p, C.b.p, (l + 1 < last && !child_zero) ? C.xp : nullptr, child_first);
    cycle_children(h, l, pre, post, shape, child_first, child_zero);
    prolong_add_level<V>(h, l, C.xp, L.xp, h->over);
    if (post > 0)
        return smooth_level(h, l, post, want_norm ? FUSE_NORM : FUSE_NONE, nullptr, false, post_slot) ? NORM_LAST_SET : NORM_NONE;
    return NORM_NONE;
}

template <typename V>
void finish_norm(Hier<V> *h, int l, int state, double *out = nullptr) {
    if (state == NORM_PLANE) {
        Level<V> &L = h->lv[l];
        launch_sum_sqrt(L.plane->partials.p, L.plane->g.n_wg, out ? out : h->norm_dev.p, h->stream);
    } else if (state == NORM_VAR7) {
        Level<V> &L = h->lv[l];
        launch_sum_sqrt(L.var7->partials.p, L.var7->n_wg, out ? out : h->norm_dev.p, h->stream);
    } else if (state == NORM_S27) {
        Level<V> &L = h->lv[l];
        Stencil27Plan<V> &P = *L.s27;
        {
            Prof<V> p(h, l, 4);
            P.norm(L.xp, L.b.p, P.have67, P.partials.p, h->stream);
        }
        launch_sum_sqrt(P.partials.p, int64_t(4) * P.g.n_wg, out ? out : h->norm_dev.p, h->stream);
    } else {
        norm_level<V>(h, l, nullptr, state == NORM_LAST_SET, out);
    }
}

template <typename V>
constexpr bool direct_io(const Level<V> &L) { return std::is_same<V, double>::value && L.ord.identity; }

template <typename V>
void ensure_nat(Hier<V> *h, int l) {
    Level<V> &L = h->lv[l];
    if (!direct_io(L) && L.nat.n < size_t(std::max<int64_t>(L.n, 1))) L.nat.alloc(std::max<int64_t>(L.n, 1));
}

// ... 23 lines not shown
        if (L.march && L.march->timed_out(h->stream))
            throw Error(OMG_ERR_HIP, "lexicographic wavefront sweep timed out waiting for a neighbouring tile's face; the iterate and "
                                     "the hand-over slots of this hierarchy are no longer consistent: destroy it and build a new one");
    if (h->plane_status.p && !have_plane_status) {
        OMG_HIP(hipMemcpyAsync(&plane_st, h->plane_status.p, sizeof(plane_st), hipMemcpyDeviceToHost, h->stream));
        OMG_HIP(hipStreamSynchronize(h->stream));
    }
    check_plane_status(h, plane_st);
}

template <typename V>
void fetch_vec(Hier<V> *h, int l, const V *src, double *host) {
    Level<V> &L = h->lv[l];
    if (direct_io(L)) {
        download_staged(host, src, size_t(L.n) * sizeof(double), h->stream);
    } else {
        ensure_nat(h, l);
        launch_scatter<V, double>(src, L.ord.identity ? nullptr : L.perm.p, L.nat.p, L.n, h->stream);
        download_staged(host, L.nat.p, size_t(L.n) * sizeof(double), h->stream);
    }
    check_march(h);
}

template <typename V>
void load_vec_dev(Hier<V> *h, int l, const double *dev, V *dst) {
    Level<V> &L = h->lv[l];
    if (direct_io(L)) OMG_HIP(hipMemcpyAsync(dst, dev, L.n * sizeof(double), hipMemcpyDeviceToDevice, h->stream));
    else launch_gather<double, V>(dev, L.ord.identity ? nullptr : L.perm.p, dst, L.n, h->stream);
}
template <typename V>
void fetch_vec_dev(Hier<V> *h, int l, const V *src, double *dev) {
    Level<V> &L = h->lv[l];
    if (direct_io(L)) OMG_HIP(hipMemcpyAsync(dev, src, L.n * sizeof(double), hipMemcpyDeviceToDevice, h->stream));
    else launch_scatter<V, double>(src, L.ord.identity ? nullptr : L.perm.p, dev, L.n, h->stream);
}

template <typename V>
double read_norm(Hier<V> *h) {
    double v = 0.0;
    uint32_t st = 0;
    OMG_HIP(hipMemcpyAsync(&v, h->norm_dev.p, sizeof(double), hipMemcpyDeviceToHost, h->stream));
    if (h->plane_status.p) OMG_HIP(hipMemcpyAsync(&st, h->plane_status.p, sizeof(st), hipMemcpyDeviceToHost, h->stream));
    OMG_HIP(hipStreamSynchronize(h->stream));
    check_march(h, true, st);
    return v;
}

template <typename V>
void drop_graph(Hier<V> *h) {
    for (auto &g : h->graphs) if (g.exec) (void)hipGraphExecDestroy(g.exec);
    h->graphs.clear();
}

template <typename V>
std::vector<V *> pointer_state(const Hier<V> *h) {
    std::vector<V *> s;
    s.reserve(2 * h->lv.size());
    for (const Level<V> &L : h->lv) { s.push_back(L.xp); s.push_back(L.tp); }
    return s;
}

template <typename V>
void run_cycle0(Hier<V> *h, int pre, int post) {
    const bool single = h->lv.size() == 1;
    auto body = [&]() {
        const int part = cycle_body(h, 0, pre, post, !single);
        if (!single) finish_norm(h, 0, part);
        else OMG_HIP(hipMemsetAsync(h->norm_dev.p, 0, sizeof(double), h->stream));
    };
    if (!h->want_graph || h->profiling) {
        body();
        return;
    }
    const std::vector<V *> cur = pointer_state(h);
    auto restore = [&](const std::vector<V *> &st) {
        for (size_t l = 0; l < h->lv.size(); ++l) { h->lv[l].xp = st[2 * l]; h->lv[l].tp = st[2 * l + 1]; }
    };
    typename Hier<V>::GraphSlot *slot = nullptr;
    for (auto &g : h->graphs)
        if (g.pre == pre && g.post == post && g.before == cur) slot = &g;
    if (!slot) {
        if (h->graphs.size() >= 2 || (!h->graphs.empty() && (h->graphs[0].pre != pre || h->graphs[0].post != post))) drop_graph(h);
        hipGraph_t g = nullptr;
        OMG_HIP(hipStreamBeginCapture(h->stream, hipStreamCaptureModeThreadLocal));
        try {
            body();
        } catch (...) {
            (void)hipStreamEndCapture(h->stream, &g);
            if (g) (void)hipGraphDestroy(g);
            restore(cur);
            throw;
        }
        OMG_HIP(hipStreamEndCapture(h->stream, &g));
        typename Hier<V>::GraphSlot ns;
        ns.pre = pre;
        ns.post = post;
        ns.before = cur;
        ns.after = pointer_state(h);
        hipError_t e = hipGraphInstantiate(&ns.exec, g, nullptr, nullptr, 0);
        (void)hipGraphDestroy(g);
        if (e != hipSuccess) {
            restore(cur);
            throw Error(OMG_ERR_HIP, std::string("hipGraphInstantiate: ") + hipGetErrorString(e));
        }
        h->graphs.push_back(std::move(ns));
        slot = &h->graphs.back();
    }
    OMG_HIP(hipGraphLaunch(slot->exec, h->stream));
    restore(slot->after);
}

template <typename V>
void check_level(const Hier<V> *h, int level) {
    OMG_REQUIRE(level >= 0 && level < (int)h->lv.size(), "level out of range");
}


template <typename V>
void build_format(Hier<V> *h, int l, const omg_csr &A, const omg_csr &R) {
    Level<V> &L = h->lv[l];
    const bool id = L.ord.identity;
    {
        HostCsr Ap;
        { SetupTimer tm("permute A"); Ap = permute_csr(A, id ? nullptr : L.ord.perm.data(), id ? nullptr : L.ord.inv.data()); }
        SetupTimer tm("encode + upload A");
        L.A.upload(Ap, L.ord.sets, h->stream);
        if (l >= 1) {
            L.diag.alloc(std::max<int64_t>(L.n, 1));
            launch_diagonal(L.A, L.diag.p, h->stream);
        }
    }
    const Ordering &co = h->lv[l + 1].ord;
    SetupTimer tm("R (and P): permute, encode, upload");
    HostCsr Rp, Rn;
    const HostCsr *r_used = &Rp;
    if (co.identity) {
        Rp = permute_csr(R, nullptr, id ? nullptr : L.ord.inv.data());
        L.R.upload(Rp, {}, h->stream);
    } else {
        Rn = permute_csr(R, nullptr, id ? nullptr : L.ord.inv.data());
        r_used = &Rn;
        L.R.upload(Rn, {}, h->stream);
    }
    {
        const char *e = getenv("OMG_PROLONG_SCATTER");
        bool ok = !(e && e[0] == '0') && L.R.all_pattern();
        if (ok) {
            std::vector<char> seen(size_t(L.n), 0);
            for (int32_t c : r_used->indices) {
                if (seen[c]) { ok = false; break; }
                seen[c] = 1;
            }
        }
        L.scatter_prolong = ok;
    }
    if (!L.scatter_prolong) {
        if (!co.identity) Rp = permute_csr(R, co.perm.data(), id ? nullptr : L.ord.inv.data());
        HostCsr Pt = transpose_csr(Rp);
        L.P.upload(Pt, {}, h->stream);
    }
    L.pw_factor = 0.0;
    L.r.alloc(L.n);
    if (h->smoother == OMG_SMOOTH_JACOBI && !L.tmp.p) { L.tmp.alloc(L.n); L.tp = L.tmp.p; }
    L.partials.alloc(L.A.n_blocks() + SUM_FOLD);
    build_plan(L);
    OMG_HIP(hipStreamSynchronize(h->stream));
}

template <typename V>
void ensure_format(Hier<V> *h, int l) {
    if (l < 0 || l >= (int)h->lv.size() || !h->lv[l].format_pending) return;
    Level<V> &L = h->lv[l];
    SetupTimer tm("plane / 27-point level: row-kernel format on first use");
    materialise_ordering(L.ord);
    if (l + 1 < (int)h->lv.size()) materialise_ordering(h->lv[l + 1].ord);
    const HostCsr A = L.s27 ? L.s27->operator_csr(h->stream) : L.var7 ? L.var7->operator_csr(h->stream) : L.plane->operator_csr();
    const HostCsr R = L.s27 ? L.s27->restriction_csr() : L.var7 ? L.var7->restriction_csr() : L.plane->restriction_csr();
    L.format_pending = false;
    build_format(h, l, view(A), view(R));
}
template <typename V>
void ensure_format(const Hier<V> *h, int l) { ensure_format(const_cast<Hier<V> *>(h), l); }


template <typename V>
std::unique_ptr<Hier<V>> create(int n_levels, const omg_csr *A, const omg_csr *R, int smoother,
                                double omega) {
    using H = Hier<V>;
    using Lv = Level<V>;
    OMG_REQUIRE(n_levels >= 1, "n_levels must be >= 1");
    OMG_REQUIRE(A != nullptr && (n_levels == 1 || R != nullptr), "A / R array is null");
// ... 945 lines not shown
            DevBuf<double> up;
            const double *dev = data;
            if (!on_device && data && nnz > 0) {
                up.alloc(size_t(nnz));
                OMG_HIP(hipMemcpyAsync(up.p, data, size_t(nnz) * sizeof(double), hipMemcpyHostToDevice, hh->stream));
                dev = up.p;
            }
            update_fine(hh, dev, nnz, true);
            mixed_update_values(hh, dev, nnz);
        });
    });
}

int omg_hierarchy_dtype(const omg_hierarchy *h, int *dtype) {
    return guarded([&] {
        OMG_REQUIRE(h && dtype, "null argument");
        *dtype = h->f ? (h->f->mixed ? OMG_DTYPE_MIXED : OMG_DTYPE_F32) : OMG_DTYPE_F64;
    });
}

int omg_hierarchy_destroy(omg_hierarchy *h) {
    return guarded([&] {
        if (!h) return;
        if (h->d || h->f) with(h, [&](auto *hh) { (void)hipStreamSynchronize(hh->stream); });
        delete h;
    });
}

int omg_hierarchy_set_stream(omg_hierarchy *h, void *hip_stream) {
    return guarded([&] {
        with(h, [&](auto *hh) {
            OMG_HIP(hipStreamSynchronize(hh->stream));
            drop_graph(hh);
            hh->stream = hip_stream ? reinterpret_cast<hipStream_t>(hip_stream) : hh->own;
        });
    });
}

int omg_hierarchy_sync(omg_hierarchy *h) {
    return guarded([&] { with(h, [&](auto *hh) { OMG_HIP(hipStreamSynchronize(hh->stream)); }); });
}

int omg_hierarchy_level_rows(const omg_hierarchy *h, int level, int64_t *n_rows) {
    return guarded([&] {
        with(h, [&](auto *hh) { check_level(hh, level); OMG_REQUIRE(n_rows, "null"); *n_rows = hh->lv[level].n; });
    });
}

int omg_hierarchy_level_sets(const omg_hierarchy *h, int level, int64_t *n_sets) {
    return guarded([&] {
        with(h, [&](auto *hh) {
            check_level(hh, level);
            OMG_REQUIRE(n_sets, "null");
            *n_sets = (int64_t)hh->lv[level].ord.sets.size() - 1;
        });
    });
}

int omg_hierarchy_level_fused(const omg_hierarchy *h, int level, int *fused) {
    return guarded([&] {
        with(h, [&](auto *hh) {
            check_level(hh, level);
            OMG_REQUIRE(fused, "null");
            ensure_format(hh, level);
            *fused = (level + 1 < (int)hh->lv.size() && can_fuse(hh, hh->lv[level])) ? 1 : 0;
        });
    });
}

int omg_hierarchy_level_flags(const omg_hierarchy *h, int level, int *flags) {
    return guarded([&] {
        with(h, [&](auto *hh) {
            check_level(hh, level);
            OMG_REQUIRE(flags, "null");
            ensure_format(hh, level);
            const bool smoothed = level + 1 < (int)hh->lv.size();
            *flags = ((smoothed && can_fuse(hh, hh->lv[level])) ? OMG_LEVEL_FUSED_LAST_SET : 0) |
                     ((smoothed && hh->lv[level].scatter_prolong) ? OMG_LEVEL_SCATTER_PROLONG : 0) |
                     ((smoothed && hh->lv[level].A.all_union()) ? OMG_LEVEL_UNION_WALK : 0) |
                     ((smoothed && hh->lv[level].march) ? OMG_LEVEL_MARCH : 0) |
                     ((smoothed && hh->lv[level].march && hh->lv[level].march->line_scan) ? OMG_LEVEL_MARCH_SCAN : 0) |
                     ((smoothed && hh->lv[level].plane && !hh->no_plane) ? OMG_LEVEL_PLANE : 0) |
                     ((smoothed && hh->lv[level].s27 && !hh->no_plane) ? OMG_LEVEL_STENCIL27 : 0) |
                     ((smoothed && hh->lv[level].var7 && !hh->no_plane) ? OMG_LEVEL_VAR7 : 0);
        });
    });
}

int omg_hierarchy_use_plane(omg_hierarchy *h, int enable) {
    return guarded([&] {
        with(h, [&](auto *hh) {
            OMG_HIP(hipStreamSynchronize(hh->stream));
            drop_graph(hh);
            hh->no_plane = enable == 0;
        });
    });
}

int omg_hierarchy_set_cycle(omg_hierarchy *h, int shape, double over_correction) {
    return guarded([&] {
        OMG_REQUIRE(shape == OMG_CYCLE_V || shape == OMG_CYCLE_F || shape == OMG_CYCLE_W, "unknown cycle shape");
        OMG_REQUIRE(std::isfinite(over_correction) && over_correction > 0.0, "the over-correction factor must be finite and positive");
        with(h, [&](auto *hh) {
            if (hh->cycle_shape == shape && hh->over == over_correction) return;
            OMG_HIP(hipStreamSynchronize(hh->stream));
            drop_graph(hh);
            hh->cycle_shape = shape;
            hh->over = over_correction;
            for (int l = 0; l + 1 < (int)hh->lv.size(); ++l) {
                auto &L = hh->lv[l];
                if (L.plane) L.plane->g.over = over_correction;
                if (L.var7) L.var7->over = over_correction;
                if (L.s27) L.s27->g.over = over_correction;
                if (!L.format_pending) ensure_prolong_values(hh, l, over_correction);
            }
        });
    });
}

int omg_hierarchy_get_cycle(const omg_hierarchy *h, int *shape, double *over_correction) {
    return guarded([&] {
        OMG_REQUIRE(shape && over_correction, "null argument");
        with(h, [&](auto *hh) { *shape = hh->cycle_shape; *over_correction = hh->over; });
    });
}

int omg_hierarchy_plane_info(const omg_hierarchy *h, int level, int64_t *out8) {
    return guarded([&] {
        with(h, [&](auto *hh) {
            check_level(hh, level);
            OMG_REQUIRE(out8, "null");
            for (int i = 0; i < 8; ++i) out8[i] = 0;
            const auto &L = hh->lv[level];
            if (!L.plane) return;
            const PlaneGeom &g = L.plane->g;
            const int64_t v[8] = {g.nx, g.ny, g.nz, g.TX, g.TY, g.LZ, g.n_wg, g.threads};
            for (int i = 0; i < 8; ++i) out8[i] = v[i];
        });
    });
}

int omg_hierarchy_set_info(const omg_hierarchy *h, int level, int set, int64_t *rows, int64_t *nnz) {
    return guarded([&] {
        with(h, [&](auto *hh) {
            check_level(hh, level);
            ensure_format(hh, level);
            const auto &A = hh->lv[level].A;
            OMG_REQUIRE(set >= 0 && size_t(set) < A.n_sets() && rows && nnz, "set out of range / null");
            *rows = A.sets[set + 1] - A.sets[set];
            *nnz = A.set_nnz[set];
        });
    });
}

int omg_hierarchy_format_info(const omg_hierarchy *h, int level, int op, int set, int64_t *out) {
    return guarded([&] {
        with(h, [&](auto *hh) {
            check_level(hh, level);
            OMG_REQUIRE(out && op >= 0 && op <= 2, "null / unknown operator");
            OMG_REQUIRE(op == 0 || level + 1 < (int)hh->lv.size(), "the coarsest level has no restriction");
            ensure_format(hh, level);
            const auto &L = hh->lv[level];
            (op == 0 ? L.A : op == 1 ? L.R : L.P).format_info(set, out);
        });
    });
}

int omg_format_selftest(const omg_csr *A, int dtype, int64_t *out) {
    return guarded([&] {
        OMG_REQUIRE(A && out, "null argument");
        OMG_REQUIRE(dtype == OMG_DTYPE_F64 || dtype == OMG_DTYPE_F32, "unknown dtype");
        validate_csr(*A, "A");
        if (dtype == OMG_DTYPE_F32) format_selftest<float>(*A, out);
        else format_selftest<double>(*A, out);
    });
}

int omg_vcycle(omg_hierarchy *h, int level, const double *b, double *x, int pre, int post,
               double *norm) {
    return guarded([&] {
        with(h, [&](auto *hh) {
            refuse_mixed(hh, "omg_vcycle");
            using V = value_of<decltype(hh)>;
            check_level(hh, level);
            OMG_REQUIRE(b && x, "b / x is null");
            OMG_REQUIRE(pre >= 0 && post >= 0, "negative sweep count");
            auto &L = hh->lv[level];
            hh->resident = false;
            load_vec(hh, level, b, L.b.p);
            load_vec(hh, level, x, L.xp);
            const int last = (int)hh->lv.size() - 1;
            const int part = cycle_body(hh, level, pre, post, level < last);
            double nv = 0.0;
            if (level < last) {
                finish_norm(hh, level, part);
                nv = read_norm(hh);
            }
            fetch_vec<V>(hh, level, L.xp, x);
            if (norm) *norm = nv;
        });
    });
}

int omg_vcycle_ex(omg_hierarchy *h, int level, const double *b, const double *x_in, double *x_out, double *x_pre,
                  int pre, int post, double *norm) {
    return guarded([&] {
// ... 659 lines not shown
```

### openmg_amd/csrc/plane.hip

```cpp
#include <algorithm>
#include <array>
#include <atomic>
#include <cmath>
#include <cstring>
#include <map>
#include <mutex>
#include <thread>
#include <type_traits>

#include "common.h"
#include "peer_wait.h"

#if defined(OMG_PLANE_STAMPS) || defined(OMG_PLANE_DBGARGS)
#define OMG_PLANE_DBG_ON 1
#endif

namespace omg {
namespace {

#ifndef PLANE_STORE_AUX
#define PLANE_STORE_AUX 2
#endif
typedef unsigned v2u __attribute__((ext_vector_type(2)));
typedef unsigned v4u __attribute__((ext_vector_type(4)));
typedef int v2i __attribute__((ext_vector_type(2)));

__device__ __forceinline__ double madd(double v, double x, double acc) { return fma(v, x, acc); }
__device__ __forceinline__ float madd(float v, float x, float acc) { return fmaf(v, x, acc); }

template <typename V>
struct P2 {
    V x, y;
};
template <typename V> struct VecOf;
template <> struct VecOf<double> {
    typedef double type __attribute__((ext_vector_type(2)));
    typedef type gtype __attribute__((aligned(8)));
};
template <> struct VecOf<float> {
    typedef float type __attribute__((ext_vector_type(2)));
    typedef type gtype __attribute__((aligned(4)));
};

__device__ __forceinline__ P2<double> bload2(__amdgpu_buffer_rsrc_t rs, int off, double) {
    const v4u q = __builtin_amdgcn_raw_buffer_load_b128(rs, off, 0, 0);
    return {__builtin_bit_cast(double, v2u{q.x, q.y}), __builtin_bit_cast(double, v2u{q.z, q.w})};
}
__device__ __forceinline__ P2<float> bload2(__amdgpu_buffer_rsrc_t rs, int off, float) {
    typedef float v2f __attribute__((ext_vector_type(2)));
    const v2f q = __builtin_bit_cast(v2f, __builtin_amdgcn_raw_buffer_load_b64(rs, off, 0, 0));
    return {q.x, q.y};
}
__device__ __forceinline__ double bload1(__amdgpu_buffer_rsrc_t rs, int off, double) {
    return __builtin_bit_cast(double, __builtin_amdgcn_raw_buffer_load_b64(rs, off, 0, 0));
}
__device__ __forceinline__ float bload1(__amdgpu_buffer_rsrc_t rs, int off, float) {
    return __builtin_bit_cast(float, __builtin_amdgcn_raw_buffer_load_b32(rs, off, 0, 0));
}
template <typename V>
__device__ __forceinline__ P2<V> lds_pair(const V *p) {
    const typename VecOf<V>::type q = *reinterpret_cast<const typename VecOf<V>::type *>(p);
    return {q.x, q.y};
}
template <typename V>
__device__ __forceinline__ void lds_put(V *p, const P2<V> &v) {
    typename VecOf<V>::type q;
    q.x = v.x;
    q.y = v.y;
    *reinterpret_cast<typename VecOf<V>::type *>(p) = q;
}
template <int AUX = PLANE_STORE_AUX>
__device__ __forceinline__ void bstore2(__amdgpu_buffer_rsrc_t rs, int off, const P2<double> &v, bool both) {
    if (both) {
        const v2u lo = __builtin_bit_cast(v2u, v.x), hi = __builtin_bit_cast(v2u, v.y);
        __builtin_amdgcn_raw_buffer_store_b128(v4u{lo.x, lo.y, hi.x, hi.y}, rs, off, 0, AUX);
    } else {
        __builtin_amdgcn_raw_buffer_store_b64(__builtin_bit_cast(v2u, v.x), rs, off, 0, AUX);
    }
}
template <int AUX = 0>
__device__ __forceinline__ void bstore2(__amdgpu_buffer_rsrc_t rs, int off, const P2<float> &v, bool both) {
    if (both) {
        __builtin_amdgcn_raw_buffer_store_b64(v2u{__builtin_bit_cast(unsigned, v.x), __builtin_bit_cast(unsigned, v.y)}, rs, off, 0, AUX);
    } else {
        __builtin_amdgcn_raw_buffer_store_b32(__builtin_bit_cast(unsigned, v.x), rs, off, 0, AUX);
    }
}
template <int AUX>
__device__ __forceinline__ void bstore1(__amdgpu_buffer_rsrc_t rs, int off, double v) {
    __builtin_amdgcn_raw_buffer_store_b64(__builtin_bit_cast(v2u, v), rs, off, 0, AUX);
}
template <int AUX>
__device__ __forceinline__ void bstore1(__amdgpu_buffer_rsrc_t rs, int off, float v) {
    __builtin_amdgcn_raw_buffer_store_b32(__builtin_bit_cast(unsigned, v), rs, off, 0, AUX);
// ... 910 lines not shown
        for (int n = 0; n < NL; ++n) {
            const int c = t + n * NT;
            const int li = c % EX, lj = (c / EX) % EY, lk = c / (EX * EY);
            if (c < vol && in_grid(i0 + li, j0 + lj, k0 + lk))
                X[c] = xv[n] + madd(a.wp, E[((lk >> 1) * CY + (lj >> 1)) * CX + (li >> 1)], V(0));
        }
        __syncthreads();
    }
    auto row = [&](int c) -> V {
        V s = madd(a.c0, X[c - EX * EY], V(0));
        s = madd(a.c1, X[c - EX], s);
        s = madd(a.c2, X[c - 1], s);
        s = madd(a.c3, X[c], s);
        s = madd(a.c4, X[c + 1], s);
        s = madd(a.c5, X[c + EX], s);
        return madd(a.c6, X[c + EX * EY], s);
    };
    auto sweep = [&](int colour, auto RING, auto FROM_ZERO) {
        constexpr int ring = decltype(RING)::value;
        constexpr int wx = BX + 2 * ring, wy = BY + 2 * ring, wz = BZ + 2 * ring, off = 2 - ring;
        constexpr int np = wx / 2 * wy * wz, NI = (np + NT - 1) / NT;
#pragma unroll
        for (int n = 0; n < NI; ++n) {
            const int p = t + n * NT;
            const int pj = (p / (wx / 2)) % wy, pk = p / (wx / 2 * wy);
            const int lj = off + pj, lk = off + pk;
            const int li = off + 2 * (p % (wx / 2)) + ((off + lj + lk + colour) & 1);
            const int gi = i0 + li, gj = j0 + lj, gk = k0 + lk;
            if (p >= np || !in_grid(gi, gj, gk)) continue;
            const int l = (lk * EY + lj) * EX + li;
            const V sum = decltype(FROM_ZERO)::value ? V(0) : row(l);
            X[l] = X[l] + block_quotient(B[l] - sum, a.c3, rc3, fast);
        }
    };
    typedef std::integral_constant<int, 0> R0;
    typedef std::integral_constant<int, 1> R1;
    typedef std::integral_constant<int, 2> R2;
    constexpr int NB = (BX * BY * BZ + NT - 1) / NT;
    if (MODE == 0) {
        if (SWEEP) {
            sweep(0, R2(), std::true_type());
            __syncthreads();
            sweep(1, R1(), std::false_type());
            __syncthreads();
        }
#pragma unroll
        for (int n = 0; n < NB; ++n) {
            const int c = t + n * NT;
            const int li = 2 + c % BX, lj = 2 + (c / BX) % BY, lk = 2 + c / (BX * BY);
            const int gi = i0 + li, gj = j0 + lj, gk = k0 + lk;
            if (c >= BX * BY * BZ || gi >= a.nx || gj >= a.ny || gk >= a.nz) continue;
            const int l = (lk * EY + lj) * EX + li;
            E[c] = B[l] - row(l);
            if (SWEEP) a.x_new[slot_of(gi, gj, gk)] = X[l];
        }
        __syncthreads();
#pragma unroll
        for (int n = 0; n < NC; ++n) {
            const int c = t + n * NT;
            if (cs[n] < 0) continue;
            const int I = c % hx, J = (c / hx) % hy, K = c / (hx * hy);
            V acc = V(0);
#pragma unroll
            for (int d = 0; d < 8; ++d)
                acc = madd(a.w, E[((2 * K + (d >> 2)) * BY + 2 * J + ((d >> 1) & 1)) * BX + 2 * I + (d & 1)], acc);
            a.bc[cs[n]] = acc;
        }
    } else {
        if (SWEEP) {
            sweep(0, R1(), std::false_type());
            __syncthreads();
            sweep(1, R0(), std::false_type());
            __syncthreads();
        }
#pragma unroll
        for (int n = 0; n < NB; ++n) {
            const int c = t + n * NT;
            const int li = 2 + c % BX, lj = 2 + (c / BX) % BY, lk = 2 + c / (BX * BY);
            const int gi = i0 + li, gj = j0 + lj, gk = k0 + lk;
            if (c >= BX * BY * BZ || gi >= a.nx || gj >= a.ny || gk >= a.nz) continue;
            a.x_new[slot_of(gi, gj, gk)] = X[(lk * EY + lj) * EX + li];
        }
    }
}

template <typename V>
struct Tile2KArgs {
    const V *x_old;
    V *x_new;
    const V *b;
    int nx, ny, nr;
    int nbx;
    V c1, c2, c3, c4, c5, w, omega;
    V wp;
    int fast_div;
    int nxc, nyc;
    const int32_t *cmap;
    V *bc;
    const V *ec;
    double *partials;
};

template <typename V, int MODE, bool XZ, bool NORM, bool SWEEP, int BX, int BY, bool JAC = false>
__global__ __launch_bounds__(256) void tile2d_kernel(const Tile2KArgs<V> a) {
    extern __shared__ __attribute__((aligned(16))) unsigned char plane_smem[];
    constexpr int EX = BX + 6, EY = BY + 6, vol = EX * EY, NT = 256;
    V *const X = reinterpret_cast<V *>(plane_smem);
    V *const B = X + vol;
    V *const XN = B + vol;
    V *const E = JAC ? XN + vol : XN;
    __shared__ double s_red[NT / 64];
    const int t = int(threadIdx.x);
    const int bi = int(blockIdx.x) % a.nbx, bj = int(blockIdx.x) / a.nbx;
    const int i0 = bi * BX - 3, j0 = bj * BY - 3;
    const V rc3 = refined_rcp(a.c3);
    const bool fast = a.fast_div != 0;
    auto slot_of = [&](int gi, int gj) { return JAC ? gj * a.nx + gi : (((gi + gj) & 1) ? a.nr : 0) + ((gj * a.nx + gi) >> 1); };
    auto in_grid = [&](int gi, int gj) { return gi >= 0 && gi < a.nx && gj >= 0 && gj < a.ny; };
    constexpr int NL = (vol + NT - 1) / NT;
    V xv[NL], bv[NL];
#pragma unroll
    for (int n = 0; n < NL; ++n) {
        const int c = t + n * NT;
        const int gi = i0 + c % EX, gj = j0 + c / EX;
        const bool ok = c < vol && in_grid(gi, gj);
        const int slot = ok ? slot_of(gi, gj) : 0;
        bv[n] = a.b[slot];
        xv[n] = XZ ? V(0) : a.x_old[slot];
        if (!ok) { bv[n] = V(0); xv[n] = V(0); }
    }
    if (MODE == 1) {
        constexpr int NC = (((EX + 1) / 2 + 1) * ((EY + 1) / 2 + 1) + NT - 1) / NT;
        constexpr int CW = (EX + 1) / 2 + 1, CH = (EY + 1) / 2 + 1;
        const int ci0 = (i0 - 1) / 2, cj0 = (j0 - 1) / 2;
#pragma unroll
        for (int n = 0; n < NC; ++n) {
            const int c = t + n * NT;
            const int I = ci0 + c % CW, J = cj0 + c / CW;
            const bool ok = c < CW * CH && I >= 0 && J >= 0 && I < a.nxc && J < a.nyc;
            const int ce = J * a.nxc + I;
            const V ev = ok ? a.ec[a.cmap ? a.cmap[ce] : ce] : V(0);
            if (c < CW * CH) E[c] = ev;
        }
        __syncthreads();
#pragma unroll
        for (int n = 0; n < NL; ++n) {
            const int c = t + n * NT;
            const int gi = i0 + c % EX, gj = j0 + c / EX;
            if (c < vol && in_grid(gi, gj)) xv[n] = xv[n] + madd(a.wp, E[((gj >> 1) - cj0) * CW + ((gi >> 1) - ci0)], V(0));
        }
        __syncthreads();
    }
#pragma unroll
    for (int n = 0; n < NL; ++n)
        if (t + n * NT < vol) { X[t + n * NT] = xv[n]; B[t + n * NT] = bv[n]; }
    __syncthreads();
    auto row_of = [&](const V *Y, int c) -> V {
        V s = madd(a.c1, Y[c - EX], V(0));
        s = madd(a.c2, Y[c - 1], s);
        s = madd(a.c3, Y[c], s);
        s = madd(a.c4, Y[c + 1], s);
        return madd(a.c5, Y[c + EX], s);
    };
    auto row = [&](int c) -> V { return row_of(X, c); };
    auto sweep = [&](int colour, auto RING) {
        constexpr int ring = decltype(RING)::value;
// ... 673 lines not shown
        }
    fprintf(stderr, "[plane stamps] %-5s ... per wave: %.1f steps, %.0f cycles entry to last step's end, %.0f of them outside the steps (100 MHz counter)\n",
            what, steps / nw, tot / nw, (tot - m - c - b - tp - sB - sC) / nw);
    fprintf(stderr, "[plane stamps] %-5s n %dx%dx%d wg %d thr %d: cycles per step and wave: wait-for-loads %.0f | top (shift, issue loads + stores) %.0f | B %.0f | C %.0f | D + rest %.0f | barrier %.0f\n",
            what, g.nx, g.ny, g.nz, g.n_wg, g.threads, m / steps, tp / steps, sB / steps, sC / steps, c / steps, b / steps);
}
#endif

template <typename K>
void allow_lds(K kernel, size_t bytes) {
    if (bytes > size_t(64) * 1024)
        OMG_HIP(hipFuncSetAttribute(reinterpret_cast<const void *>(kernel), hipFuncAttributeMaxDynamicSharedMemorySize, int(bytes)));
}

}

template <typename V>
void peer_args(PlaneKArgs<V> &k, const typename PlanePlan<V>::Peer &p, hipStream_t s) {
    for (int i = 0; i < 2; ++i) { k.peer_x[i] = p.x[i]; k.peer_bc[i] = p.bc[i]; k.peer_flag[i] = p.flag[i]; }
    k.peer_shift = int(p.shift); k.peer_cshift = int(p.cshift);
    OMG_REQUIRE(p.planes == PEER_PLANES && (p.cplanes == PEER_CPLANES || (!p.bc[0] && !p.bc[1])), "plane pass with neighbours: three planes of x, two of the coarse right-hand side");
    for (int i = 0; i < 4; ++i) { k.wait_flag[i] = p.wait_flag[i]; k.wait_seq[i] = p.wait_seq[i]; }
    k.fused_wait = p.fused_wait ? 1 : 0;
    k.done = p.done; k.flag_seq = p.seq; k.status = p.status; k.spin = p.spin;
    OMG_REQUIRE(p.done, "plane pass with neighbours: no workgroup counter");
    if (!p.fused_wait && (p.wait_flag[0] || p.wait_flag[1] || p.wait_flag[2] || p.wait_flag[3])) {
        hipLaunchKernelGGL(plane_wait_kernel, dim3(1), dim3(64), 0, s, p.wait_flag[0], p.wait_flag[1], p.wait_flag[2], p.wait_flag[3],
                           p.wait_seq[0], p.wait_seq[1], p.wait_seq[2], p.wait_seq[3], p.status, p.spin);
        OMG_HIP(hipGetLastError());
    }
}

struct BlockGeom {
    int shape, BX, BY, BZ, nbx, nby, nbz, threads;
    size_t lds;
};
inline bool block_level(const PlaneGeom &g) { return g.block; }
constexpr int BLOCK_SHAPES[4][3] = {{16, 8, 8}, {8, 8, 8}, {8, 4, 4}, {4, 4, 4}};
inline BlockGeom choose_block(const PlaneGeom &g, size_t value_bytes) {
    BlockGeom k;
    int pick = 3;
    for (int i = 0; i < 4; ++i) {
        const int64_t n = int64_t((g.nx + BLOCK_SHAPES[i][0] - 1) / BLOCK_SHAPES[i][0]) * ((g.ny + BLOCK_SHAPES[i][1] - 1) / BLOCK_SHAPES[i][1]) *
                          ((g.nz + BLOCK_SHAPES[i][2] - 1) / BLOCK_SHAPES[i][2]);
        if (n >= 128) { pick = i; break; }
    }
    k.shape = pick;
    k.BX = BLOCK_SHAPES[pick][0]; k.BY = BLOCK_SHAPES[pick][1]; k.BZ = BLOCK_SHAPES[pick][2];
    k.nbx = (g.nx + k.BX - 1) / k.BX; k.nby = (g.ny + k.BY - 1) / k.BY; k.nbz = (g.nz + k.BZ - 1) / k.BZ;
    const size_t vol = size_t(k.BX + 4) * size_t(k.BY + 4) * size_t(k.BZ + 4);
    k.threads = vol >= 1024 ? 256 : 128;
    k.lds = (2 * vol + std::max(size_t(k.BX) * k.BY * k.BZ, vol / 8)) * value_bytes;
    return k;
}
template <typename V, int MODE, int S, bool SWEEP>
void launch_block_shape(const BlockGeom &k, const BlockKArgs<V> &a, hipStream_t s) {
    auto kernel = block_kernel<V, MODE, BLOCK_SHAPES[S][0], BLOCK_SHAPES[S][1], BLOCK_SHAPES[S][2], SWEEP>;
    allow_lds(kernel, k.lds);
    hipLaunchKernelGGL(kernel, dim3(unsigned(k.nbx * k.nby * k.nbz)), dim3(unsigned(k.threads)), k.lds, s, a);
}
template <typename V, int MODE, bool SWEEP = true>
void launch_block(const PlaneGeom &g, const V *x_old, V *x_new, const V *b, const typename PlanePlan<V>::Coarse &c, hipStream_t s) {
    const BlockGeom k = choose_block(g, sizeof(V));
    BlockKArgs<V> a;
    std::memset(&a, 0, sizeof(a));
    a.x_old = x_old; a.x_new = x_new; a.b = b;
    a.nx = g.nx; a.ny = g.ny; a.nz = g.nz; a.nr = int(int64_t(g.nx) * g.ny * g.nz / 2);
    a.nbx = k.nbx; a.nby = k.nby;
    a.c0 = V(g.c[0]); a.c1 = V(g.c[1]); a.c2 = V(g.c[2]); a.c3 = V(g.c[3]); a.c4 = V(g.c[4]); a.c5 = V(g.c[5]); a.c6 = V(g.c[6]);
    a.w = V(g.w);
    a.wp = V(g.over * g.w);
    a.fast_div = (std::fabs(g.c[3]) >= 0x1p-400 && std::fabs(g.c[3]) <= 0x1p400) ? 1 : 0;
    a.nxc = g.nx / 2; a.nyc = g.ny / 2;
    a.cmap = c.map; a.bc = c.b; a.ec = c.e;
    switch (k.shape) {
        case 0: launch_block_shape<V, MODE, 0, SWEEP>(k, a, s); break;
        case 1: launch_block_shape<V, MODE, 1, SWEEP>(k, a, s); break;
        case 2: launch_block_shape<V, MODE, 2, SWEEP>(k, a, s); break;
        default: launch_block_shape<V, MODE, 3, SWEEP>(k, a, s); break;
    }
    OMG_HIP(hipGetLastError());
}


template <typename V, int MODE, bool XZ, bool NORM, bool SWEEP>
void launch_tile2d(const PlaneGeom &g, const V *x_old, V *x_new, const V *b, const typename PlanePlan<V>::Coarse &c, double *out, hipStream_t s) {
    Tile2KArgs<V> a;
    std::memset(&a, 0, sizeof(a));
    a.x_old = x_old; a.x_new = x_new; a.b = b;
    a.nx = g.nx; a.ny = g.ny; a.nr = int(int64_t(g.nx) * g.ny / 2);
    a.nbx = g.ntx;
    a.c1 = V(g.c[1]); a.c2 = V(g.c[2]); a.c3 = V(g.c[3]); a.c4 = V(g.c[4]); a.c5 = V(g.c[5]);
    a.w = V(g.w);
    a.wp = V(g.over * g.w);
    a.omega = V(g.omega);
    a.fast_div = (std::fabs(g.c[3]) >= 0x1p-400 && std::fabs(g.c[3]) <= 0x1p400) ? 1 : 0;
    a.nxc = g.nx / 2; a.nyc = g.ny / 2;
    a.cmap = c.map; a.bc = c.b; a.ec = c.e;
    a.partials = out;
    auto go = [&](auto kernel) {
        allow_lds(kernel, g.lds_bytes);
        hipLaunchKernelGGL(kernel, dim3(unsigned(g.n_wg)), dim3(256), g.lds_bytes, s, a);
    };
    if (g.jacobi) {
        if (g.TX == 64) go(tile2d_kernel<V, MODE, XZ, NORM, SWEEP, 64, 32, true>);
        else if (g.TX == 32) go(tile2d_kernel<V, MODE, XZ, NORM, SWEEP, 32, 16, true>);
        else go(tile2d_kernel<V, MODE, XZ, NORM, SWEEP, 16, 8, true>);
    } else {
        if (g.TX == 64) go(tile2d_kernel<V, MODE, XZ, NORM, SWEEP, 64, 32>);
        else if (g.TX == 32) go(tile2d_kernel<V, MODE, XZ, NORM, SWEEP, 32, 16>);
        else go(tile2d_kernel<V, MODE, XZ, NORM, SWEEP, 16, 8>);
    }
    OMG_HIP(hipGetLastError());
}

inline bool small_tile(const PlaneGeom &g) { return g.la2 && g.threads <= 128; }

template <typename V>
int plane_part(const PlaneGeom &g, PlaneKArgs<V> &k, int part) {
    const int nxy = g.ntx * g.nty, nzo = g.z_end - g.z_base;
    if (part == 0) return g.n_wg;
    if (part == 1) {
        k.zc_base = g.z_base; k.zc_stride = nzo - PLANE_EDGE; k.zc_len = PLANE_EDGE; k.zc_end = g.z_end; k.part_slot0 = 0;
        return 2 * nxy;
    }
    k.zc_base = g.z_base + PLANE_EDGE; k.zc_stride = g.LZ; k.zc_len = g.LZ; k.zc_end = g.z_end - PLANE_EDGE; k.part_slot0 = 2 * nxy;
    return nxy * ((nzo - 2 * PLANE_EDGE + g.LZ - 1) / g.LZ);
}
template <typename K, typename V>
void launch_plane(K kernel, const PlaneGeom &g, const PlaneKArgs<V> &k, hipStream_t s, int n_wg = -1) {
    if (n_wg == 0) return;
    allow_lds(kernel, g.lds_bytes);
    hipLaunchKernelGGL(kernel, dim3(unsigned(n_wg < 0 ? g.n_wg : n_wg)), dim3(unsigned(g.threads)), g.lds_bytes, s, k);
    OMG_HIP(hipGetLastError());
}

template <typename V>
int plane_gate(const PlaneGeom &g, PlaneKArgs<V> &k, const typename PlanePlan<V>::Gate &gate, int lz) {
    const int nxy = g.ntx * g.nty, nzo = g.z_end - g.z_base;
    k.zc_base = g.z_base + PLANE_EDGE; k.zc_stride = lz; k.zc_len = lz; k.zc_end = g.z_end - PLANE_EDGE; k.part_slot0 = 0;
    k.edge_wg0 = nxy * ((nzo - 2 * PLANE_EDGE + lz - 1) / lz);
    for (int i = 0; i < 4; ++i) { k.wait_flag[i] = gate.flag[i]; k.wait_seq[i] = gate.seq[i]; }
    k.spin = gate.spin;
    if (gate.status) k.status = gate.status;
    return k.edge_wg0 + 2 * nxy;
}

template <typename V>
int PlanePlan<V>::gate_lz() const {
    const int nxy = g.ntx * g.nty, nzo = g.z_end - g.z_base;
    static const int forced = [] { const char *e = experiment_env("OMG_PLANE_GATE_LZ"); return e ? atoi(e) : 0; }();
    if (forced >= 2) return forced / 2 * 2;
    const int chunks = std::max(1, (256 - (2 * nxy * 5 + 5) / 6) / nxy);
    const int lz = ((nzo - 2 * PLANE_EDGE + chunks - 1) / chunks + 1) / 2 * 2;
    return std::max(lz, g.LZ);
}

template <typename V>
int PlanePlan<V>::gate_partials() const {
    const int nxy = g.ntx * g.nty, nzo = g.z_end - g.z_base;
    return can_split() ? nxy * (2 + (nzo - 2 * PLANE_EDGE + gate_lz() - 1) / gate_lz()) : g.n_wg;
}

template <typename V>
void PlanePlan<V>::down(const V *x_old, V *x_new, const V *b, bool x_zero, const Coarse &c, hipStream_t s, const Peer *peer, bool sweep, int part,
                        const Gate *gate) const {
// ... 141 lines not shown
```

Before: 3748.

## Fuse coarsest sine solve with the up-sweeps of the last one or two levels

Adds a tail kernel in which every workgroup redundantly runs the 16^3 MFMA sine-transform coarse solve in LDS. It then prolongs and post-smooths one or two plane levels (32^3 and 64^3) inside the same launch, replacing separate coarse-solve and plane-up launches at the bottom of the V-cycle. The aim is to remove the launch and serialisation overhead of the tiny coarse levels. In exchange, each block repeats the coarse solve and uses more LDS per workgroup.

After: 3940 (median of 6 runs). 1.05x the previous value.

```diff
diff --git a/include/openmg_hip.h b/include/openmg_hip.h
--- a/include/openmg_hip.h
+++ b/include/openmg_hip.h
@@ -63,7 +63,9 @@
 #define OMG_LEVEL_PLANE            64
 #define OMG_LEVEL_VAR7             256
 #define OMG_LEVEL_STENCIL27        128
+#define OMG_LEVEL_TAIL_FUSED       1024
 int omg_hierarchy_level_flags(const omg_hierarchy *h, int level, int *flags);
+int omg_hierarchy_tail_info(const omg_hierarchy *h, int64_t *out2);
 int omg_hierarchy_use_plane(omg_hierarchy *h, int enable);
 #define OMG_CYCLE_V 0
 #define OMG_CYCLE_F 1
diff --git a/openmg_amd/_hip.py b/openmg_amd/_hip.py
--- a/openmg_amd/_hip.py
+++ b/openmg_amd/_hip.py
@@ -60,6 +60,7 @@
     "omg_hierarchy_set_info": (_I, [_P, _I, _I, _I64P, _I64P]),
     "omg_hierarchy_level_fused": (_I, [_P, _I, _IP]),
     "omg_hierarchy_level_flags": (_I, [_P, _I, _IP]),
+    "omg_hierarchy_tail_info": (_I, [_P, _I64P]),
     "omg_hierarchy_use_plane": (_I, [_P, _I]),
     "omg_hierarchy_set_cycle": (_I, [_P, _I, _D]),
     "omg_hierarchy_get_cycle": (_I, [_P, _IP, _DP]),
@@ -481,7 +482,12 @@
         check(lib().omg_hierarchy_level_flags(self._h, int(level), ctypes.byref(f)))
         return {"fused_last_set": bool(f.value & 1), "scatter_prolong": bool(f.value & 2), "union_walk": bool(f.value & 16),
                 "march": bool(f.value & 32), "plane": bool(f.value & 64), "stencil27": bool(f.value & 128), "var7": bool(f.value & 256),
-                "march_scan": bool(f.value & 512)}
+                "march_scan": bool(f.value & 512), "tail_fused": bool(f.value & 1024)}
+
+    def tail_info(self):
+        out = (ctypes.c_int64 * 2)()
+        check(lib().omg_hierarchy_tail_info(self._h, out))
+        return int(out[0]), int(out[1])
 
     def use_plane(self, enable=True):
         check(lib().omg_hierarchy_use_plane(self._h, 1 if enable else 0))
diff --git a/openmg_amd/csrc/coarse.hip b/openmg_amd/csrc/coarse.hip
--- a/openmg_amd/csrc/coarse.hip
+++ b/openmg_amd/csrc/coarse.hip
@@ -4,6 +4,7 @@
 #include <type_traits>
 
 #include "common.h"
+#include "sine_cube16.h"
 
 namespace omg {
 namespace {
@@ -185,7 +186,6 @@
 }
 
 constexpr int SINE_THREADS = 1024;
-typedef double v4d __attribute__((ext_vector_type(4)));
 template <typename V, int E>
 __global__ __launch_bounds__(SINE_THREADS) void sine_solve_kernel(const V *__restrict__ b, V *__restrict__ x, int nx, int ny, int nz,
                                                                  const double *__restrict__ tables, const double *__restrict__ lambda) {
@@ -262,65 +262,12 @@
         if (place[q] >= 0) x[int(threadIdx.x) + q * SINE_THREADS] = V(sine_buf[place[q]]);
 }
 
-__device__ __forceinline__ void wave_lds_exchange() {
-    __builtin_amdgcn_fence(__ATOMIC_RELEASE, "wavefront");
-    __builtin_amdgcn_wave_barrier();
-    __builtin_amdgcn_fence(__ATOMIC_ACQUIRE, "wavefront");
-}
-
 template <typename V>
 __global__ __launch_bounds__(SINE_THREADS) void sine_cube16_kernel(const V *__restrict__ b, V *__restrict__ x, const double *__restrict__ tables,
                                                                    const double *__restrict__ lambda) {
-    constexpr int N = 16, PX = N + 1;
-    __shared__ double buf[N * N * PX];
-    const int lane = int(threadIdx.x) & 63, w = int(threadIdx.x) >> 6;
-    const int c = lane & 15, k4 = lane >> 4;
-    double sx[4], sy[4], sz[4], lam[4], rhs[4];
-#pragma unroll
-    for (int ks = 0; ks < 4; ++ks) {
-        sx[ks] = tables[(0 * N + c) * N + 4 * ks + k4];
-        sy[ks] = tables[(1 * N + c) * N + 4 * ks + k4];
-        sz[ks] = tables[(2 * N + c) * N + 4 * ks + k4];
-        rhs[ks] = double(b[(w * N + c) * N + 4 * ks + k4]);
-        lam[ks] = lambda[((4 * ks + k4) * N + w) * N + c];
-    }
-    auto transform = [&](const double (&S)[4], const double (&in)[4]) -> v4d {
-        v4d acc = {0.0, 0.0, 0.0, 0.0};
-#pragma unroll
-        for (int ks = 0; ks < 4; ++ks) acc = __builtin_amdgcn_mfma_f64_16x16x4f64(S[ks], in[ks], acc, 0, 0, 0);
-        return acc;
-    };
-    double in[4];
-    v4d acc = transform(sx, rhs);
-#pragma unroll
-    for (int r = 0; r < 4; ++r) buf[(w * N + c) * PX + 4 * r + k4] = acc[r];
-    wave_lds_exchange();
-#pragma unroll
-    for (int ks = 0; ks < 4; ++ks) in[ks] = buf[(w * N + 4 * ks + k4) * PX + c];
-    acc = transform(sy, in);
-#pragma unroll
-    for (int r = 0; r < 4; ++r) buf[(w * N + 4 * r + k4) * PX + c] = acc[r];
-    __syncthreads();
-#pragma unroll
-    for (int ks = 0; ks < 4; ++ks) in[ks] = buf[((4 * ks + k4) * N + w) * PX + c];
-    acc = transform(sz, in);
-#pragma unroll
-    for (int r = 0; r < 4; ++r) in[r] = acc[r] / lam[r];
-    acc = transform(sz, in);
-#pragma unroll
-    for (int r = 0; r < 4; ++r) buf[((4 * r + k4) * N + w) * PX + c] = acc[r];
-    __syncthreads();
-#pragma unroll
-    for (int ks = 0; ks < 4; ++ks) in[ks] = buf[(w * N + c) * PX + 4 * ks + k4];
-    acc = transform(sx, in);
-#pragma unroll
-    for (int r = 0; r < 4; ++r) buf[(w * N + c) * PX + 4 * r + k4] = acc[r];
-    wave_lds_exchange();
-#pragma unroll
-    for (int ks = 0; ks < 4; ++ks) in[ks] = buf[(w * N + 4 * ks + k4) * PX + c];
-    acc = transform(sy, in);
-#pragma unroll
-    for (int r = 0; r < 4; ++r) x[(w * N + 4 * r + k4) * N + c] = V(acc[r]);
+    __shared__ double buf[SINE16_BUF];
+    const Sine16Operands o = sine_cube16_load(b, tables, lambda);
+    sine_cube16_solve(o, buf, [&](int i, int j, int k, double v) { x[(k * SINE16_N + j) * SINE16_N + i] = V(v); });
 }
 
 bool detect_symmetric_star(const HostCsr &A, int64_t &nx, int64_t &ny, int64_t &nz, double (&c)[4]) {
@@ -683,13 +630,18 @@
 }
 
 template <typename V>
+bool CoarseSolver<V>::cube16() const {
+    static const bool on = [] { const char *e = experiment_env("OMG_SINE_CUBE16"); return !(e && e[0] == '0'); }();
+    return n != 0 && P == 0 && sx == 16 && sy == 16 && sz == 16 && on;
+}
+
+template <typename V>
 void CoarseSolver<V>::solve(const V *b, V *x, hipStream_t s) const {
     if (n == 0) return;
     if (P == 0) {
         const int E = std::max(sx, std::max(sy, sz)) <= 16 ? 16 : 32;
         const size_t lds = (size_t(sx + 1) * size_t(sy) * size_t(sz) + 2 + size_t(sx + sy + sz) * size_t(E)) * sizeof(double);
-        static const bool cube16 = [] { const char *e = experiment_env("OMG_SINE_CUBE16"); return !(e && e[0] == '0'); }();
-        if (E == 16 && sx == 16 && sy == 16 && sz == 16 && cube16) {
+        if (cube16()) {
             hipLaunchKernelGGL((sine_cube16_kernel<V>), dim3(1), dim3(SINE_THREADS), 0, s, b, x, sine.p, lambda.p);
         } else if (E == 16) {
             hipLaunchKernelGGL((sine_solve_kernel<V, 16>), dim3(1), dim3(SINE_THREADS), lds, s, b, x, sx, sy, sz, sine.p, lambda.p);
diff --git a/openmg_amd/csrc/common.h b/openmg_amd/csrc/common.h
--- a/openmg_amd/csrc/common.h
+++ b/openmg_amd/csrc/common.h
@@ -501,6 +501,7 @@
     void build(const HostCsr &A, hipStream_t s);
     bool build_sine(const HostCsr &A, hipStream_t s);
     void solve(const V *b, V *x, hipStream_t s) const;
+    bool cube16() const;
 };
 
 constexpr int MARCH_FACE_PAD = 72;
@@ -624,6 +625,21 @@
 };
 
 template <typename V>
+struct TailUp {
+    const PlaneGeom *top = nullptr, *mid = nullptr;
+    const V *x_old = nullptr, *b = nullptr, *mid_x_old = nullptr, *mid_b = nullptr;
+    V *x_new = nullptr, *mid_x_new = nullptr;
+    const int32_t *cmap = nullptr;
+    const V *cb = nullptr;
+    V *cx = nullptr;
+    const double *tables = nullptr, *lambda = nullptr;
+    bool sweep = true;
+};
+bool tail_up_level(const PlaneGeom &g, int nxc, int nyc, int nzc);
+template <typename V>
+void launch_tail_up(const TailUp<V> &u, hipStream_t s);
+
+template <typename V>
 struct Var7Plan {
     int nx = 0, ny = 0, nz = 0;
     double w = 0.0;
diff --git a/openmg_amd/csrc/hierarchy.hip b/openmg_amd/csrc/hierarchy.hip
--- a/openmg_amd/csrc/hierarchy.hip
+++ b/openmg_amd/csrc/hierarchy.hip
@@ -187,10 +187,13 @@
     bool resident = false;
     bool no_fuse = [] { const char *e = getenv("OMG_NO_FUSE"); return e && e[0] == '1'; }();
     bool no_plane = false;
+    int64_t tail_launches = 0, tail_replayed = 0;
+    int tail_fuse = [] { const char *e = getenv("OMG_TAIL_FUSE"); return (e && e[0] >= '0' && e[0] <= '2' && !e[1]) ? e[0] - '0' : 2; }();
     struct GraphSlot {
         hipGraphExec_t exec = nullptr;
         int pre = -1, post = -1;
         std::vector<V *> before, after;
+        int64_t tail = 0;
     };
     bool want_graph = false;
     std::vector<GraphSlot> graphs;
@@ -677,6 +680,48 @@
         cycle_body(h, l + 1, pre, post, false, nullptr, false, nullptr, false, shape == OMG_CYCLE_F ? OMG_CYCLE_V : OMG_CYCLE_W);
 }
 
+struct PlaneDown { bool child_first, child_zero; };
+template <typename V>
+PlaneDown plane_down_half(Hier<V> *h, int l, int pre, int post, bool x_zero, bool first_done, int halves, typename PlanePlan<V>::Coarse &c) {
+    const int last = (int)h->lv.size() - 1;
+    Level<V> &L = h->lv[l];
+    Level<V> &C = h->lv[l + 1];
+    if (pre > 1) smooth_level(h, l, pre - 1, FUSE_NONE, nullptr, first_done);
+    const bool child_plane = l + 1 < last && use_plane(h, C, pre, post);
+    const bool child_zero = child_plane && pre <= 1 && halves == 3;
+    if (l + 1 < last && !child_zero) ensure_format(h, l + 1);
+    const bool child_first = l + 1 < last && !child_zero && !use_s27(h, C) && !L.plane->g.dim2 && first_sweep_in_restrict(h, C, pre);
+    c.map = L.r_out.p;
+    c.b = C.b.p;
+    c.x = (l + 1 < last && !child_zero) ? C.xp : nullptr;
+    c.diag = child_first ? C.diag.p : nullptr;
+    c.first_end = child_first ? int(C.A.sets[1]) : 0;
+    if (child_zero && pre == 0) OMG_HIP(hipMemsetAsync(C.xp, 0, size_t(C.n) * sizeof(V), h->stream));
+    {
+        Prof<V> p(h, l, 5);
+        L.plane->down(L.xp, L.tp, L.b.p, x_zero, c, h->stream, nullptr, pre >= 1);
+    }
+    if (pre >= 1) std::swap(L.xp, L.tp);
+    if (l == h->pre_level) OMG_HIP(hipMemcpyAsync(h->pre_buf.p, L.xp, size_t(L.n) * sizeof(V), hipMemcpyDeviceToDevice, h->stream));
+    return {child_first, child_zero};
+}
+
+template <typename V>
+int tail_fuse_depth(const Hier<V> *h, int l, int post, int shape) {
+    const int last = (int)h->lv.size() - 1;
+    if (h->tail_fuse <= 0 || shape != OMG_CYCLE_V || h->cycle_shape != OMG_CYCLE_V || post > 1 || l < 0 || l >= last || !h->coarse.cube16()) return 0;
+    auto fits = [&](int k) {
+        const Level<V> &K = h->lv[k];
+        if (!use_plane(h, K, 1, post)) return false;
+        const Level<V> &D = h->lv[k + 1];
+        if (k + 1 == last) return tail_up_level(K.plane->g, 16, 16, 16);
+        return use_plane(h, D, 1, post) && tail_up_level(K.plane->g, D.plane->g.nx, D.plane->g.ny, D.plane->g.nz);
+    };
+    if (l == last - 1) return fits(l) ? 1 : 0;
+    if (l == last - 2 && h->tail_fuse >= 2) return fits(l) && fits(l + 1) ? 2 : 0;
+    return 0;
+}
+
 template <typename V>
 int cycle_body(Hier<V> *h, int l, int pre, int post, bool want_norm, double *pre_slot, bool first_done, double *post_slot, bool x_zero,
                int shape) {
@@ -757,27 +802,34 @@
         return smooth_level(h, l, post, want_norm ? FUSE_NORM : FUSE_NONE, nullptr, false, post_slot) ? NORM_LAST_SET : NORM_NONE;
     }
     if (use_plane(h, L, pre, post)) {
-        if (pre > 1) smooth_level(h, l, pre - 1, FUSE_NONE, nullptr, first_done);
-        const bool child_plane = l + 1 < last && use_plane(h, C, pre, post);
-        const bool child_zero = child_plane && pre <= 1 && halves == 3;
-        if (l + 1 < last && !child_zero) ensure_format(h, l + 1);
-        const bool child_first = l + 1 < last && !child_zero && !use_s27(h, C) && !L.plane->g.dim2 && first_sweep_in_restrict(h, C, pre);
         typename PlanePlan<V>::Coarse c;
-        c.map = L.r_out.p;
-        c.b = C.b.p;
-        c.x = (l + 1 < last && !child_zero) ? C.xp : nullptr;
-        c.diag = child_first ? C.diag.p : nullptr;
-        c.first_end = child_first ? int(C.A.sets[1]) : 0;
-        if (child_zero && pre == 0) OMG_HIP(hipMemsetAsync(C.xp, 0, size_t(C.n) * sizeof(V), h->stream));
-        {
-            Prof<V> p(h, l, 5);
-            L.plane->down(L.xp, L.tp, L.b.p, x_zero, c, h->stream, nullptr, pre >= 1);
-        }
-        if (pre >= 1) std::swap(L.xp, L.tp);
-        if (l == h->pre_level) OMG_HIP(hipMemcpyAsync(h->pre_buf.p, L.xp, size_t(L.n) * sizeof(V), hipMemcpyDeviceToDevice, h->stream));
-        cycle_children(h, l, pre, post, shape, child_first, child_zero);
+        const PlaneDown d = plane_down_half(h, l, pre, post, x_zero, first_done, halves, c);
+        double *out = (want_norm && post <= 1) ? (post_slot ? post_slot : L.plane->partials.p) : nullptr;
+        const int fuse = halves == 3 && !out ? tail_fuse_depth(h, l, post, shape) : 0;
+        if (fuse) {
+            TailUp<V> u;
+            u.top = &L.plane->g; u.x_old = L.xp; u.x_new = L.tp; u.b = L.b.p;
+            u.cmap = L.r_out.p;
+            if (fuse == 2) {
+                typename PlanePlan<V>::Coarse cc;
+                plane_down_half(h, l + 1, pre, post, d.child_zero, d.child_first, halves, cc);
+                u.mid = &C.plane->g; u.mid_x_old = C.xp; u.mid_x_new = C.tp; u.mid_b = C.b.p;
+                u.cmap = C.r_out.p;
+            }
+            Level<V> &Z = h->lv[last];
+            u.cb = Z.b.p; u.cx = Z.xp; u.tables = h->coarse.sine.p; u.lambda = h->coarse.lambda.p;
+            u.sweep = post >= 1;
+            {
+                Prof<V> p(h, l, 6);
+                launch_tail_up<V>(u, h->stream);
+                ++h->tail_launches;
+            }
+            if (fuse == 2) std::swap(C.xp, C.tp);
+            std::swap(L.xp, L.tp);
+            return NORM_NONE;
+        }
+        cycle_children(h, l, pre, post, shape, d.child_first, d.child_zero);
         c.e = C.xp;
-        double *out = (want_norm && post <= 1) ? (post_slot ? post_slot : L.plane->partials.p) : nullptr;
         {
             Prof<V> p(h, l, 6);
             L.plane->up(L.xp, L.tp, L.b.p, c, out, h->stream, nullptr, post >= 1);
@@ -967,6 +1019,7 @@
     if (!slot) {
         if (h->graphs.size() >= 2 || (!h->graphs.empty() && (h->graphs[0].pre != pre || h->graphs[0].post != post))) drop_graph(h);
         hipGraph_t g = nullptr;
+        const int64_t tail_before = h->tail_launches;
         OMG_HIP(hipStreamBeginCapture(h->stream, hipStreamCaptureModeThreadLocal));
         try {
             body();
@@ -982,6 +1035,8 @@
         ns.post = post;
         ns.before = cur;
         ns.after = pointer_state(h);
+        ns.tail = h->tail_launches - tail_before;
+        h->tail_launches = tail_before;
         hipError_t e = hipGraphInstantiate(&ns.exec, g, nullptr, nullptr, 0);
         (void)hipGraphDestroy(g);
         if (e != hipSuccess) {
@@ -992,6 +1047,8 @@
         slot = &h->graphs.back();
     }
     OMG_HIP(hipGraphLaunch(slot->exec, h->stream));
+    h->tail_launches += slot->tail;
+    h->tail_replayed += slot->tail;
     restore(slot->after);
 }
 
@@ -2103,7 +2160,9 @@
                      ((smoothed && hh->lv[level].march && hh->lv[level].march->line_scan) ? OMG_LEVEL_MARCH_SCAN : 0) |
                      ((smoothed && hh->lv[level].plane && !hh->no_plane) ? OMG_LEVEL_PLANE : 0) |
                      ((smoothed && hh->lv[level].s27 && !hh->no_plane) ? OMG_LEVEL_STENCIL27 : 0) |
-                     ((smoothed && hh->lv[level].var7 && !hh->no_plane) ? OMG_LEVEL_VAR7 : 0);
+                     ((smoothed && hh->lv[level].var7 && !hh->no_plane) ? OMG_LEVEL_VAR7 : 0) |
+                     ((tail_fuse_depth(hh, level, 1, hh->cycle_shape) || tail_fuse_depth(hh, level - 1, 1, hh->cycle_shape) == 2)
+                          ? OMG_LEVEL_TAIL_FUSED : 0);
         });
     });
 }
@@ -2143,6 +2202,13 @@
     return guarded([&] {
         OMG_REQUIRE(shape && over_correction, "null argument");
         with(h, [&](auto *hh) { *shape = hh->cycle_shape; *over_correction = hh->over; });
+    });
+}
+
+int omg_hierarchy_tail_info(const omg_hierarchy *h, int64_t *out2) {
+    return guarded([&] {
+        OMG_REQUIRE(out2, "null");
+        with(h, [&](auto *hh) { out2[0] = hh->tail_launches; out2[1] = hh->tail_replayed; });
     });
 }
 
diff --git a/openmg_amd/csrc/plane.hip b/openmg_amd/csrc/plane.hip
--- a/openmg_amd/csrc/plane.hip
+++ b/openmg_amd/csrc/plane.hip
@@ -10,6 +10,7 @@
 
 #include "common.h"
 #include "peer_wait.h"
+#include "sine_cube16.h"
 
 #if defined(OMG_PLANE_STAMPS) || defined(OMG_PLANE_DBGARGS)
 #define OMG_PLANE_DBG_ON 1
@@ -1086,6 +1087,163 @@
             a.x_new[slot_of(gi, gj, gk)] = X[(lk * EY + lj) * EX + li];
         }
     }
+}
+
+template <typename V>
+struct TailLevelArgs {
+    const V *x_old;
+    V *x_new;
+    const V *b;
+    int nx, ny, nz, nr;
+    V c0, c1, c2, c3, c4, c5, c6;
+    V wp;
+    int fast_div;
+};
+template <typename V>
+struct TailKArgs {
+    TailLevelArgs<V> top, mid;
+    int nbx, nby;
+    const int32_t *cmap;
+    const V *cb;
+    V *cx;
+    const double *tables, *lambda;
+};
+constexpr int TAIL_BX = 16, TAIL_BY = 8, TAIL_BZ = 8, TAIL_THREADS = 1024;
+
+template <typename V, int RX, int RY, int RZ>
+struct TailRegion {
+    static constexpr int vol = RX * RY * RZ, NT = TAIL_THREADS, NL = (vol + NT - 1) / NT;
+    const TailLevelArgs<V> &a;
+    const int oi, oj, ok;
+    V xv[NL], bv[NL];
+    int ps[NL];
+    __device__ __forceinline__ TailRegion(const TailLevelArgs<V> &lv, int i, int j, int k) : a(lv), oi(i), oj(j), ok(k) {}
+    __device__ __forceinline__ bool in_grid(int gi, int gj, int gk) const {
+        return gi >= 0 && gi < a.nx && gj >= 0 && gj < a.ny && gk >= 0 && gk < a.nz;
+    }
+    __device__ __forceinline__ int slot_of(int gi, int gj, int gk) const {
+        return (((gi + gj + gk) & 1) ? a.nr : 0) + (((gk * a.ny + gj) * a.nx + gi) >> 1);
+    }
+    __device__ __forceinline__ void load() {
+        const int t = int(threadIdx.x);
+#pragma unroll
+        for (int n = 0; n < NL; ++n) {
+            const int c = t + n * NT;
+            const int gi = oi + c % RX, gj = oj + (c / RX) % RY, gk = ok + c / (RX * RY);
+            const bool in = c < vol && in_grid(gi, gj, gk);
+            const int slot = in ? slot_of(gi, gj, gk) : 0;
+            bv[n] = a.b[slot];
+            xv[n] = a.x_old[slot];
+            if (!in) { bv[n] = V(0); xv[n] = V(0); }
+        }
+    }
+    __device__ __forceinline__ void parents_in_cube16(const int32_t *cmap) {
+        const int t = int(threadIdx.x);
+#pragma unroll
+        for (int n = 0; n < NL; ++n) {
+            const int c = t + n * NT;
+            const int gi = oi + c % RX, gj = oj + (c / RX) % RY, gk = ok + c / (RX * RY);
+            const int ce = (c < vol && in_grid(gi, gj, gk)) ? ((gk >> 1) * SINE16_N + (gj >> 1)) * SINE16_N + (gi >> 1) : 0;
+            ps[n] = cmap ? cmap[ce] : ce;
+        }
+    }
+    template <bool SWEEP, typename PARENT>
+    __device__ __forceinline__ void up(V *X, V *B, PARENT parent) {
+        const int t = int(threadIdx.x);
+#pragma unroll
+        for (int n = 0; n < NL; ++n) {
+            const int c = t + n * NT;
+            const int gi = oi + c % RX, gj = oj + (c / RX) % RY, gk = ok + c / (RX * RY);
+            if (c >= vol) continue;
+            V x = xv[n];
+            if (in_grid(gi, gj, gk)) x = xv[n] + madd(a.wp, parent(n, gi >> 1, gj >> 1, gk >> 1), V(0));
+            X[c] = x;
+            B[c] = bv[n];
+        }
+        __syncthreads();
+        if (!SWEEP) return;
+        const V rc3 = refined_rcp(a.c3);
+        const bool fast = a.fast_div != 0;
+        auto row = [&](int c) -> V {
+            V s = madd(a.c0, X[c - RX * RY], V(0));
+            s = madd(a.c1, X[c - RX], s);
+            s = madd(a.c2, X[c - 1], s);
+            s = madd(a.c3, X[c], s);
+            s = madd(a.c4, X[c + 1], s);
+            s = madd(a.c5, X[c + RX], s);
+            return madd(a.c6, X[c + RX * RY], s);
+        };
+#pragma unroll
+        for (int colour = 0; colour < 2; ++colour) {
+            const int ring = 1 - colour, off = 2 - ring;
+            const int wx = RX - 2 * off, wy = RY - 2 * off, wz = RZ - 2 * off;
+            const int np = wx / 2 * wy * wz;
+#pragma unroll
+            for (int n = 0; n < ((RX - 2) / 2 * (RY - 2) * (RZ - 2) + NT - 1) / NT; ++n) {
+                const int p = t + n * NT;
+                const int lj = off + (p / (wx / 2)) % wy, lk = off + p / (wx / 2 * wy);
+                const int l0 = off + 2 * (p % (wx / 2));
+                const int li = l0 + ((oi + l0 + oj + lj + ok + lk + colour) & 1);
+                const int gi = oi + li, gj = oj + lj, gk = ok + lk;
+                if (p >= np || !in_grid(gi, gj, gk)) continue;
+                const int l = (lk * RY + lj) * RX + li;
+                X[l] = X[l] + block_quotient(B[l] - row(l), a.c3, rc3, fast);
+            }
+            __syncthreads();
+        }
+    }
+    template <int CX, int CY, int CZ>
+    __device__ __forceinline__ void store(const V *X, int fx, int fy, int fz) const {
+        const int t = int(threadIdx.x);
+#pragma unroll
+        for (int n = 0; n < (CX * CY * CZ + NT - 1) / NT; ++n) {
+            const int c = t + n * NT;
+            const int li = fx + c % CX, lj = fy + (c / CX) % CY, lk = fz + c / (CX * CY);
+            const int gi = oi + li, gj = oj + lj, gk = ok + lk;
+            if (c >= CX * CY * CZ || !in_grid(gi, gj, gk)) continue;
+            a.x_new[slot_of(gi, gj, gk)] = X[(lk * RY + lj) * RX + li];
+        }
+    }
+};
+
+template <typename V, int DEPTH, bool SWEEP>
+__global__ __launch_bounds__(TAIL_THREADS) void tail_up_kernel(const TailKArgs<V> a) {
+    extern __shared__ __attribute__((aligned(16))) unsigned char plane_smem[];
+    constexpr int BX = TAIL_BX, BY = TAIL_BY, BZ = TAIL_BZ;
+    typedef TailRegion<V, BX + 4, BY + 4, BZ + 4> Top;
+    typedef TailRegion<V, BX / 2 + 6, BY / 2 + 6, BZ / 2 + 6> Mid;
+    constexpr int MX = BX / 2 + 6, MY = BY / 2 + 6;
+    constexpr int N = SINE16_N, PX = SINE16_PX;
+    double *const sol = reinterpret_cast<double *>(plane_smem);
+    V *const X = reinterpret_cast<V *>(sol + SINE16_BUF);
+    V *const B = X + Top::vol;
+    V *const XM = B + Top::vol;
+    V *const BM = XM + Mid::vol;
+    const int bi = int(blockIdx.x) % a.nbx, bj = (int(blockIdx.x) / a.nbx) % a.nby, bk = int(blockIdx.x) / (a.nbx * a.nby);
+    const Sine16Operands so = sine_cube16_load(a.cb, a.tables, a.lambda);
+    Top top(a.top, bi * BX - 2, bj * BY - 2, bk * BZ - 2);
+    Mid mid(a.mid, bi * (BX / 2) - 3, bj * (BY / 2) - 3, bk * (BZ / 2) - 3);
+    top.load();
+    if (DEPTH == 2) mid.load();
+    if (DEPTH == 2) mid.parents_in_cube16(a.cmap);
+    else top.parents_in_cube16(a.cmap);
+    const bool first = blockIdx.x == 0;
+    sine_cube16_solve(so, sol, [&](int i, int j, int k, double v) {
+        const V r = V(v);
+        if (first) a.cx[(k * N + j) * N + i] = r;
+        sol[(k * N + j) * PX + i] = double(r);
+    });
+    __syncthreads();
+    auto solved = [&](int slot) -> V { return V(sol[(slot / (N * N) * N + slot / N % N) * PX + slot % N]); };
+    if (DEPTH == 2) {
+        mid.template up<SWEEP>(XM, BM, [&](int n, int, int, int) -> V { return solved(mid.ps[n]); });
+        mid.template store<BX / 2, BY / 2, BZ / 2>(XM, 3, 3, 3);
+        const int mi = mid.oi, mj = mid.oj, mk = mid.ok;
+        top.template up<SWEEP>(X, B, [&](int, int I, int J, int K) -> V { return XM[((K - mk) * MY + (J - mj)) * MX + (I - mi)]; });
+    } else {
+        top.template up<SWEEP>(X, B, [&](int n, int, int, int) -> V { return solved(top.ps[n]); });
+    }
+    top.template store<BX, BY, BZ>(X, 2, 2, 2);
 }
 
 template <typename V>
@@ -1925,6 +2083,56 @@
     OMG_HIP(hipGetLastError());
 }
 
+template <typename V>
+TailLevelArgs<V> tail_level(const PlaneGeom &g, const V *x_old, V *x_new, const V *b) {
+    TailLevelArgs<V> a;
+    std::memset(&a, 0, sizeof(a));
+    a.x_old = x_old; a.x_new = x_new; a.b = b;
+    a.nx = g.nx; a.ny = g.ny; a.nz = g.nz; a.nr = int(int64_t(g.nx) * g.ny * g.nz / 2);
+    a.c0 = V(g.c[0]); a.c1 = V(g.c[1]); a.c2 = V(g.c[2]); a.c3 = V(g.c[3]); a.c4 = V(g.c[4]); a.c5 = V(g.c[5]); a.c6 = V(g.c[6]);
+    a.wp = V(g.over * g.w);
+    a.fast_div = (std::fabs(g.c[3]) >= 0x1p-400 && std::fabs(g.c[3]) <= 0x1p400) ? 1 : 0;
+    return a;
+}
+template <typename V, int DEPTH, bool SWEEP>
+void launch_tail_kernel(const TailKArgs<V> &a, int wgs, hipStream_t s) {
+    const size_t cells = size_t(TAIL_BX + 4) * (TAIL_BY + 4) * (TAIL_BZ + 4) +
+                         (DEPTH == 2 ? size_t(TAIL_BX / 2 + 6) * (TAIL_BY / 2 + 6) * (TAIL_BZ / 2 + 6) : 0);
+    const size_t lds = SINE16_BUF * sizeof(double) + 2 * cells * sizeof(V);
+    auto kernel = tail_up_kernel<V, DEPTH, SWEEP>;
+    allow_lds(kernel, lds);
+    hipLaunchKernelGGL(kernel, dim3(unsigned(wgs)), dim3(TAIL_THREADS), lds, s, a);
+    OMG_HIP(hipGetLastError());
+}
+
+bool tail_up_level(const PlaneGeom &g, int nxc, int nyc, int nzc) {
+    return g.block && !g.dim2 && !g.jacobi && g.z_base == 0 && g.z_end == g.nz && g.nx == 2 * nxc && g.ny == 2 * nyc && g.nz == 2 * nzc;
+}
+
+template <typename V>
+void launch_tail_up(const TailUp<V> &u, hipStream_t s) {
+    const PlaneGeom &g = *u.top;
+    OMG_REQUIRE(u.mid ? tail_up_level(g, u.mid->nx, u.mid->ny, u.mid->nz) && tail_up_level(*u.mid, SINE16_N, SINE16_N, SINE16_N)
+                      : tail_up_level(g, SINE16_N, SINE16_N, SINE16_N),
+                "fused tail: block levels of twice the extents of the level below, above a 16 x 16 x 16 coarsest grid");
+    TailKArgs<V> a;
+    std::memset(&a, 0, sizeof(a));
+    a.top = tail_level<V>(g, u.x_old, u.x_new, u.b);
+    if (u.mid) a.mid = tail_level<V>(*u.mid, u.mid_x_old, u.mid_x_new, u.mid_b);
+    a.nbx = (g.nx + TAIL_BX - 1) / TAIL_BX; a.nby = (g.ny + TAIL_BY - 1) / TAIL_BY;
+    const int wgs = a.nbx * a.nby * ((g.nz + TAIL_BZ - 1) / TAIL_BZ);
+    a.cmap = u.cmap; a.cb = u.cb; a.cx = u.cx; a.tables = u.tables; a.lambda = u.lambda;
+    if (u.mid) {
+        if (u.sweep) launch_tail_kernel<V, 2, true>(a, wgs, s);
+        else launch_tail_kernel<V, 2, false>(a, wgs, s);
+    } else {
+        if (u.sweep) launch_tail_kernel<V, 1, true>(a, wgs, s);
+        else launch_tail_kernel<V, 1, false>(a, wgs, s);
+    }
+}
+template void launch_tail_up<double>(const TailUp<double> &, hipStream_t);
+template void launch_tail_up<float>(const TailUp<float> &, hipStream_t);
+
 
 template <typename V, int MODE, bool XZ, bool NORM, bool SWEEP>
 void launch_tile2d(const PlaneGeom &g, const V *x_old, V *x_new, const V *b, const typename PlanePlan<V>::Coarse &c, double *out, hipStream_t s) {
diff --git a/openmg_amd/csrc/sine_cube16.h b/openmg_amd/csrc/sine_cube16.h
--- /dev/null
+++ b/openmg_amd/csrc/sine_cube16.h
@@ -0,0 +1,82 @@
+#pragma once
+#include <hip/hip_runtime.h>
+
+namespace omg {
+
+typedef double v4d __attribute__((ext_vector_type(4)));
+
+__device__ __forceinline__ void wave_lds_exchange() {
+    __builtin_amdgcn_fence(__ATOMIC_RELEASE, "wavefront");
+    __builtin_amdgcn_wave_barrier();
+    __builtin_amdgcn_fence(__ATOMIC_ACQUIRE, "wavefront");
+}
+
+constexpr int SINE16_N = 16, SINE16_PX = SINE16_N + 1;
+constexpr int SINE16_BUF = SINE16_N * SINE16_N * SINE16_PX;
+
+struct Sine16Operands {
+    double sx[4], sy[4], sz[4], lam[4], rhs[4];
+};
+template <typename V>
+__device__ __forceinline__ Sine16Operands sine_cube16_load(const V *__restrict__ b, const double *__restrict__ tables,
+                                                           const double *__restrict__ lambda) {
+    constexpr int N = SINE16_N;
+    const int lane = int(threadIdx.x) & 63, w = int(threadIdx.x) >> 6;
+    const int c = lane & 15, k4 = lane >> 4;
+    Sine16Operands o;
+#pragma unroll
+    for (int ks = 0; ks < 4; ++ks) {
+        o.sx[ks] = tables[(0 * N + c) * N + 4 * ks + k4];
+        o.sy[ks] = tables[(1 * N + c) * N + 4 * ks + k4];
+        o.sz[ks] = tables[(2 * N + c) * N + 4 * ks + k4];
+        o.rhs[ks] = double(b[(w * N + c) * N + 4 * ks + k4]);
+        o.lam[ks] = lambda[((4 * ks + k4) * N + w) * N + c];
+    }
+    return o;
+}
+
+template <typename OUT>
+__device__ __forceinline__ void sine_cube16_solve(const Sine16Operands &o, double *buf, OUT out) {
+    constexpr int N = SINE16_N, PX = SINE16_PX;
+    const int lane = int(threadIdx.x) & 63, w = int(threadIdx.x) >> 6;
+    const int c = lane & 15, k4 = lane >> 4;
+    auto transform = [&](const double (&S)[4], const double (&in)[4]) -> v4d {
+        v4d acc = {0.0, 0.0, 0.0, 0.0};
+#pragma unroll
+        for (int ks = 0; ks < 4; ++ks) acc = __builtin_amdgcn_mfma_f64_16x16x4f64(S[ks], in[ks], acc, 0, 0, 0);
+        return acc;
+    };
+    double in[4];
+    v4d acc = transform(o.sx, o.rhs);
+#pragma unroll
+    for (int r = 0; r < 4; ++r) buf[(w * N + c) * PX + 4 * r + k4] = acc[r];
+    wave_lds_exchange();
+#pragma unroll
+    for (int ks = 0; ks < 4; ++ks) in[ks] = buf[(w * N + 4 * ks + k4) * PX + c];
+    acc = transform(o.sy, in);
+#pragma unroll
+    for (int r = 0; r < 4; ++r) buf[(w * N + 4 * r + k4) * PX + c] = acc[r];
+    __syncthreads();
+#pragma unroll
+    for (int ks = 0; ks < 4; ++ks) in[ks] = buf[((4 * ks + k4) * N + w) * PX + c];
+    acc = transform(o.sz, in);
+#pragma unroll
+    for (int r = 0; r < 4; ++r) in[r] = acc[r] / o.lam[r];
+    acc = transform(o.sz, in);
+#pragma unroll
+    for (int r = 0; r < 4; ++r) buf[((4 * r + k4) * N + w) * PX + c] = acc[r];
+    __syncthreads();
+#pragma unroll
+    for (int ks = 0; ks < 4; ++ks) in[ks] = buf[(w * N + c) * PX + 4 * ks + k4];
+    acc = transform(o.sx, in);
+#pragma unroll
+    for (int r = 0; r < 4; ++r) buf[(w * N + c) * PX + 4 * r + k4] = acc[r];
+    wave_lds_exchange();
+#pragma unroll
+    for (int ks = 0; ks < 4; ++ks) in[ks] = buf[(w * N + 4 * ks + k4) * PX + c];
+    acc = transform(o.sy, in);
+#pragma unroll
+    for (int r = 0; r < 4; ++r) out(c, 4 * r + k4, w, acc[r]);
+}
+
+}
```
